# jsyrjala/zraytrace

Measured on AMD Instinct MI355X. Metric: Mrays/s + achieved HBM GB/s, bunny BVH @ 2048², 1024spp, 1/2/4/8 GPUs, higher is better.
Workload: dtype f32

## Files before the change

include/zrt.h:

```cpp
#ifndef ZRT_H
#define ZRT_H

#include <stddef.h>
#include <stdint.h>

#ifdef __cplusplus
extern "C" {
#endif

#define ZRT_ABI_VERSION 2

enum {
  ZRT_OK = 0,
  ZRT_E_INVALID = -1,
  ZRT_E_NOMEM = -2,
  ZRT_E_HIP = -3,
  ZRT_E_UNSUPPORTED = -4,
  ZRT_E_NODEVICE = -5,
  ZRT_E_IO = -6,
  ZRT_E_PARSE = -7
};

enum { ZRT_PRIM_SPHERE = 0, ZRT_PRIM_TRIANGLE = 1 };
enum { ZRT_MAT_LAMBERTIAN = 0, ZRT_MAT_METAL = 1, ZRT_MAT_DIELECTRIC = 2 };
// ... 245 lines not shown
                        const zrt_adaptive* adaptive);
int zrt_ctx_adapt_level(zrt_ctx* ctx, float* dev_tiles, void* hip_stream, zrt_level_info* out);
int zrt_ctx_adapt_samples(zrt_ctx* ctx, uint32_t* per_tile, uint32_t cap_tiles);

typedef int (*zrt_level_fn)(void* user, const float* rgb, const zrt_level_info* info);
int zrt_render_adaptive(const zrt_scene* scene, const zrt_camera* camera, const zrt_params* params,
                        const zrt_adaptive* adaptive, zrt_level_fn on_level, void* user, float* out_rgb,
                        uint32_t* out_samples, zrt_stats* stats);
int zrt_render_adaptive_progress(const zrt_scene* scene, const zrt_camera* camera, const zrt_params* params,
                                 const zrt_adaptive* adaptive, zrt_level_fn on_level, void* user, float* out_rgb,
                                 uint32_t* out_samples, zrt_stats* stats, zrt_scanline* scanlines);

int zrt_debug_adapt_plan(const zrt_params* params, const zrt_adaptive* adaptive, uint32_t* levels,
                         uint32_t cap, uint32_t* n_levels);

int zrt_ctx_accum_variance(zrt_ctx* ctx, float* dev_tiles_var, void* hip_stream);

int zrt_ctx_assemble_plane(zrt_ctx* ctx, const zrt_params* params, const float* dev_gathered,
                           uint32_t stride_tiles, float* dev_frame, void* hip_stream);

typedef struct zrt_variance_plan {
  uint32_t chunk;
  uint32_t k;
  float ik;
  float sc;
} zrt_variance_plan;
int zrt_debug_variance_plan(const zrt_params* params, uint32_t n_samples, zrt_variance_plan* out);

typedef struct zrt_denoise {
  uint32_t iterations;
  float sigma_color;
  float sigma_normal;
  float sigma_albedo;
  float sigma_depth;
  uint32_t reserved[3];
} zrt_denoise;
enum { ZRT_DEFAULT_DENOISE_ITERATIONS = 5u };

int zrt_denoise_defaults(zrt_denoise* out);

int zrt_ctx_features(zrt_ctx* ctx, const zrt_camera* camera, const zrt_params* params,
                     float* dev_features, void* hip_stream);

int zrt_ctx_denoise(zrt_ctx* ctx, const zrt_params* params, const zrt_denoise* dn,
                    const float* dev_frame, const float* dev_features,
                    float* dev_out, void* hip_stream);
int zrt_ctx_denoise_ms(zrt_ctx* ctx, double* ms);

int zrt_render_denoised(const zrt_scene* scene, const zrt_camera* camera, const zrt_params* params,
                        const zrt_adaptive* adaptive, const zrt_denoise* dn, float* out_rgb, float* out_noisy,
                        float* out_features, zrt_stats* stats, double* denoise_ms);

enum { ZRT_DN_DEMODULATE = 1u };

int zrt_denoise_guided_defaults(zrt_denoise* out, uint32_t* flags);

int zrt_ctx_denoise_guided(zrt_ctx* ctx, const zrt_params* params, const zrt_denoise* dn, uint32_t flags,
                           const float* dev_frame, const float* dev_features, const float* dev_variance,
                           float* dev_out, float* dev_out_variance, void* hip_stream);

int zrt_render_denoised_guided(const zrt_scene* scene, const zrt_camera* camera, const zrt_params* params,
                               const zrt_adaptive* adaptive, const zrt_denoise* dn, uint32_t flags, float* out_rgb,
                               float* out_noisy, float* out_features, float* out_variance, zrt_stats* stats,
                               double* denoise_ms);

typedef struct zrt_reproject_plan {
  zrt_vec3 origin;
  zrt_vec3 rn, ru, rv;
  float s;
  uint32_t valid;
} zrt_reproject_plan;
int zrt_debug_reproject_plan(const zrt_camera* prev, const zrt_params* params, zrt_reproject_plan* out);

typedef struct zrt_temporal {
  float alpha_min;
  uint32_t max_history;
  float sigma_normal;
  float sigma_depth;
  uint32_t flags;
  uint32_t reserved[3];
} zrt_temporal;
enum { ZRT_TA_DEMODULATE = 1u };
enum { ZRT_DEFAULT_TEMPORAL_HISTORY = 32u };

int zrt_temporal_defaults(zrt_temporal* out);

int zrt_ctx_temporal(zrt_ctx* ctx, const zrt_camera* camera, const zrt_params* params, const zrt_temporal* tp,
                     const float* dev_frame, const float* dev_features, const float* dev_variance,
                     float* dev_out, float* dev_out_variance, uint32_t* dev_out_len, void* hip_stream);
int zrt_ctx_temporal_reset(zrt_ctx* ctx);
int zrt_ctx_temporal_ms(zrt_ctx* ctx, double* ms);

typedef int (*zrt_frame_fn)(void* user, const float* rgb, uint32_t frame);
int zrt_render_temporal(const zrt_scene* scene, const zrt_camera* cameras, uint32_t n_frames,
                        const zrt_params* params, const zrt_temporal* tp, const zrt_denoise* dn, uint32_t dn_flags,
                        zrt_frame_fn on_frame, void* user, float* out_rgb, zrt_stats* stats);

typedef struct zrt_scene_data zrt_scene_data;

int zrt_scene_load(uint32_t scene_index, const char* assets_dir,
                   zrt_scene_data** out, zrt_camera* camera);
const zrt_scene* zrt_scene_view(const zrt_scene_data* data);
void zrt_scene_free(zrt_scene_data* data);

int zrt_scene_write(const zrt_scene* scene, const zrt_camera* camera, const char* path);
int zrt_scene_read(const char* path, zrt_scene_data** out, zrt_camera* camera);

int zrt_obj_read(const char* path, uint32_t material, zrt_prim** out_prims, uint32_t* n_prims);
void zrt_free(void* p);

int zrt_image_read_png(const char* path, uint32_t* width, uint32_t* height, float** out_pixels);
int zrt_image_write_png(const char* path, const float* rgb, uint32_t width, uint32_t height);
int zrt_image_write_ppm(const char* path, const float* rgb, uint32_t width, uint32_t height);

typedef struct zrt_bvh_node {
  zrt_vec3 min;
  int32_t left;
  zrt_vec3 max;
  int32_t right;
} zrt_bvh_node;

int zrt_bvh_build(const zrt_scene* scene, zrt_bvh_node** out_nodes,
                  uint32_t* n_nodes, uint32_t* max_depth);

int zrt_bvh_build_device(const zrt_scene* scene, uint32_t device, zrt_bvh_node** out_nodes,
                         uint32_t* n_nodes, uint32_t* max_depth);

int zrt_debug_math(int fn, const float* x, const float* y, float* out, uint32_t n, uint32_t device);
int zrt_debug_rng(uint32_t prng, uint64_t key, uint64_t* out, uint32_t n, uint32_t device);
int zrt_debug_division(uint64_t n, uint64_t* counts, uint32_t device);
int zrt_debug_compact(const uint32_t* list, uint32_t n, const uint32_t* tile_done, uint32_t n_tiles,
                      uint32_t* out, uint32_t* count, uint32_t device);
int zrt_debug_lds_plans(const zrt_scene* scene, uint32_t* n_checked);
int zrt_debug_buffer_plans(const zrt_scene* scene, uint32_t legacy, uint32_t* n_checked);
typedef struct zrt_launch_plan {
  uint32_t mode;
  uint32_t kmode;
  uint32_t sampling_loop;
  uint32_t stk16;
  uint32_t wf, pool, qnodes, guard_on;
  uint32_t stack_depth;
  uint32_t stack_rows;
  uint32_t att_rows;
  uint32_t att_rows_per_path;
  uint32_t mats_in_lds;
  uint32_t lds_bytes;
  uint64_t ovf_bytes_per_lane;
} zrt_launch_plan;
int zrt_debug_launch_plan(const zrt_scene* scene, const zrt_params* params, zrt_launch_plan* out);
int zrt_debug_lean_kernel(const zrt_scene* scene, const zrt_camera* camera, const zrt_params* params,
                          uint32_t* lean);
int zrt_debug_qnodes(const zrt_scene* scene, uint64_t* n_checked);
int zrt_debug_octant_offsets(uint32_t stride_f4, uint32_t n_top, uint32_t node_f4);

#ifdef __cplusplus
}
#endif
#endif
```

zraytrace_amd/__init__.py:

```python
from __future__ import annotations

import ctypes as C
import os
from dataclasses import dataclass

import numpy as np

from . import _ffi
from ._ffi import (ZRT_PRNG_XOROSHIRO128, ZRT_PRNG_XOSHIRO256, ZRT_RNG_COUNTER,
                   ZRT_RNG_REFERENCE_STREAM, ZRT_TRAVERSAL_FAST, ZRT_TRAVERSAL_REFERENCE,
                   ZRT_TRAVERSAL_BINARY, ZRT_FLAG_STATS, ZRT_FLAG_NO_SCHEDULE, ZRT_FLAG_SCANLINES, ZRT_FLAG_GUARD,
                   ZRT_DN_DEMODULATE, ZRT_TA_DEMODULATE, ZrtError, check)

REPO = os.path.dirname(os.path.dirname(os.path.abspath(__file__)))
ASSETS = os.path.join(REPO, "assets")

SCENES = {0: "manAndBall", 1: "threeBalls", 2: "bunnyAndBall", 3: "teapotAndBall",
          4: "teapotAndBallCircle", 5: "goat"}


def lib():
    return _ffi.load()


# ... 471 lines not shown
    def debug_counters(self, n: int = 48):
        out = (C.c_uint64 * n)()
        check(lib().zrt_ctx_debug_counters(self._h, out, n))
        return list(out)

    def debug_wave_times(self, cap: int = 1 << 16):
        out = np.zeros(cap, np.uint64)
        n = C.c_uint32()
        check(lib().zrt_ctx_debug_wave_times(self._h, out.ctypes.data_as(C.POINTER(C.c_uint64)), cap, C.byref(n)))
        return out[: 2 * n.value].reshape(-1, 2).copy()

    def debug_schedule(self, cap: int = 1 << 20):
        costs = np.zeros(cap, np.uint32)
        order = np.zeros(cap, np.uint32)
        n = C.c_uint32()
        check(lib().zrt_ctx_debug_schedule(self._h, costs.ctypes.data_as(C.POINTER(C.c_uint32)),
                                           order.ctypes.data_as(C.POINTER(C.c_uint32)), cap, C.byref(n)))
        return costs[: n.value].copy(), order[: n.value].copy()

    def kernel_ms(self) -> float:
        ms = C.c_double()
        check(lib().zrt_ctx_last_kernel_ms(self._h, C.byref(ms)))
        return ms.value

    def close(self):
        if getattr(self, "_h", None):
            lib().zrt_ctx_destroy(self._h)
            self._h = None

    def __del__(self):
        try:
            self.close()
        except Exception:
            pass


def bvh_build(scene):
    view = scene.view if isinstance(scene, LoadedScene) else scene
    nodes = C.POINTER(_ffi.BvhNode)()
    n = C.c_uint32()
    depth = C.c_uint32()
    check(lib().zrt_bvh_build(view, C.byref(nodes), C.byref(n), C.byref(depth)))
    try:
        return nodes_to_numpy(nodes, n.value) + (depth.value,)
    finally:
        lib().zrt_free(C.cast(nodes, C.c_void_p))


def bvh_build_device(scene, device: int = 0):
    view = scene.view if isinstance(scene, LoadedScene) else scene
    nodes = C.POINTER(_ffi.BvhNode)()
    n = C.c_uint32()
    depth = C.c_uint32()
    check(lib().zrt_bvh_build_device(view, device, C.byref(nodes), C.byref(n), C.byref(depth)))
    try:
        return nodes_to_numpy(nodes, n.value) + (depth.value,)
    finally:
        lib().zrt_free(C.cast(nodes, C.c_void_p))


def nodes_to_numpy(nodes, n):
    dt = np.dtype([("min", "<f4", 3), ("left", "<i4"), ("max", "<f4", 3), ("right", "<i4")])
    buf = np.ctypeslib.as_array(C.cast(nodes, C.POINTER(C.c_uint8)), shape=(n * 32,)).copy()
    a = buf.view(dt)
    return a["min"].copy(), a["max"].copy(), a["left"].copy(), a["right"].copy()


def debug_division(n: int = 1 << 30, device: int = 0) -> dict:
    out = (C.c_uint64 * 5)()
    check(lib().zrt_debug_division(n, out, device))
    return dict(zip(("rcp_sqrt_all_2p32", "div", "unit", "inv_dir", "jitter"), (int(v) for v in out)))


def debug_math(fn: int, x, y=None, device: int = 0):
    x = np.ascontiguousarray(x, dtype=np.float32)
    out = np.empty_like(x)
    yp = None
    if y is not None:
        y = np.ascontiguousarray(y, dtype=np.float32)
        yp = y.ctypes.data_as(C.POINTER(C.c_float))
    check(lib().zrt_debug_math(fn, x.ctypes.data_as(C.POINTER(C.c_float)), yp,
                               out.ctypes.data_as(C.POINTER(C.c_float)), x.size, device))
    return out


def debug_rng(prng: int, key: int, n: int, device: int = 0):
    out = np.empty(n, dtype=np.uint64)
    check(lib().zrt_debug_rng(prng, key, out.ctypes.data_as(C.POINTER(C.c_uint64)), n, device))
    return out


def debug_compact(list_, tile_done, fill: int = 0xFFFFFFFF, device: int = 0):
    u32p = C.POINTER(C.c_uint32)
    lst = np.ascontiguousarray(list_, dtype=np.uint32)
    done = np.ascontiguousarray(tile_done, dtype=np.uint32)
    out = np.full(lst.size, fill, dtype=np.uint32)
    count = C.c_uint32()
    check(lib().zrt_debug_compact(lst.ctypes.data_as(u32p), lst.size, done.ctypes.data_as(u32p), done.size,
                                  out.ctypes.data_as(u32p), C.byref(count), device))
    return out, count.value


def read_png(path: str):
    w, h, px = C.c_uint32(), C.c_uint32(), C.POINTER(C.c_float)()
    check(lib().zrt_image_read_png(path.encode(), C.byref(w), C.byref(h), C.byref(px)))
    try:
        return np.ctypeslib.as_array(px, shape=(h.value, w.value, 3)).copy()
    finally:
        lib().zrt_free(px)


def write_png(path: str, image) -> None:
    img = np.ascontiguousarray(image, dtype=np.float32)
    h, w, _ = img.shape
    check(lib().zrt_image_write_png(os.fsencode(path), img.ctypes.data_as(C.POINTER(C.c_float)), w, h))


def write_ppm(path: str, image) -> None:
    img = np.ascontiguousarray(image, dtype=np.float32)
    h, w, _ = img.shape
    check(lib().zrt_image_write_ppm(os.fsencode(path), img.ctypes.data_as(C.POINTER(C.c_float)), w, h))


def debug_lds_plans(scene) -> int:
    view = scene.view if isinstance(scene, LoadedScene) else scene
    n = C.c_uint32()
    check(lib().zrt_debug_lds_plans(view, C.byref(n)))
    return n.value


def debug_buffer_plans(scene, legacy: bool = False) -> int:
    view = scene.view if isinstance(scene, LoadedScene) else scene
    n = C.c_uint32()
    check(lib().zrt_debug_buffer_plans(view, 1 if legacy else 0, C.byref(n)))
    return n.value


def debug_launch_plan(scene, params) -> dict:
    view = scene.view if isinstance(scene, LoadedScene) else scene
    out = _ffi.LaunchPlan()
    p = params.abi()
    check(lib().zrt_debug_launch_plan(view, C.byref(p), C.byref(out)))
    return out.as_dict()


def debug_lean_kernel(scene, camera, params) -> bool:
    view = scene.view if isinstance(scene, LoadedScene) else scene
    out = C.c_uint32()
    p = params.abi()
    check(lib().zrt_debug_lean_kernel(view, C.byref(camera), C.byref(p), C.byref(out)))
    return bool(out.value)


def debug_qnodes(scene) -> int:
    view = scene.view if isinstance(scene, LoadedScene) else scene
    n = C.c_uint64()
    check(lib().zrt_debug_qnodes(view, C.byref(n)))
    return n.value


def debug_octant_offsets(stride_f4: int, n_top: int, node_f4: int = 8) -> None:
    check(lib().zrt_debug_octant_offsets(stride_f4, n_top, node_f4))
```

zraytrace_amd/_ffi.py:

```python
from __future__ import annotations

import ctypes as C
import os

HERE = os.path.dirname(os.path.abspath(__file__))
LIB_PATH = os.environ.get("ZRT_LIB") or os.path.join(HERE, "libzrt.so")

ABI_VERSION = 2
ZRT_OK = 0
ZRT_E_INVALID = -1
ZRT_E_NOMEM = -2
ZRT_E_HIP = -3
ZRT_E_UNSUPPORTED = -4
ZRT_E_NODEVICE = -5
ZRT_E_IO = -6
ZRT_E_PARSE = -7

ZRT_PRIM_SPHERE, ZRT_PRIM_TRIANGLE = 0, 1
ZRT_MAT_LAMBERTIAN, ZRT_MAT_METAL, ZRT_MAT_DIELECTRIC = 0, 1, 2
ZRT_TEX_COLOR, ZRT_TEX_IMAGE = 0, 1
ZRT_RNG_COUNTER, ZRT_RNG_REFERENCE_STREAM = 0, 1
ZRT_PRNG_XOROSHIRO128, ZRT_PRNG_XOSHIRO256 = 0, 1
ZRT_TRAVERSAL_FAST, ZRT_TRAVERSAL_REFERENCE, ZRT_TRAVERSAL_BINARY = 0, 1, 2
ZRT_FLAG_STATS = 1
# ... 123 lines not shown
                ("reserved2", C.c_uint32)]

    def as_dict(self):
        return {name: getattr(self, name) for name, _ in self._fields_ if not name.startswith("reserved")}


LEVEL_FN = C.CFUNCTYPE(C.c_int, C.c_void_p, C.POINTER(C.c_float), C.POINTER(LevelInfo))


class Denoise(C.Structure):
    _fields_ = [("iterations", C.c_uint32), ("sigma_color", C.c_float), ("sigma_normal", C.c_float),
                ("sigma_albedo", C.c_float), ("sigma_depth", C.c_float), ("reserved", C.c_uint32 * 3)]

    def as_dict(self):
        return {name: getattr(self, name) for name, _ in self._fields_ if name != "reserved"}


class VariancePlan(C.Structure):
    _fields_ = [("chunk", C.c_uint32), ("k", C.c_uint32), ("ik", C.c_float), ("sc", C.c_float)]

    def as_dict(self):
        return {name: getattr(self, name) for name, _ in self._fields_}


class ReprojectPlan(C.Structure):
    _fields_ = [("origin", Vec3), ("rn", Vec3), ("ru", Vec3), ("rv", Vec3), ("s", C.c_float), ("valid", C.c_uint32)]


class Temporal(C.Structure):
    _fields_ = [("alpha_min", C.c_float), ("max_history", C.c_uint32), ("sigma_normal", C.c_float),
                ("sigma_depth", C.c_float), ("flags", C.c_uint32), ("reserved", C.c_uint32 * 3)]

    def as_dict(self):
        return {name: getattr(self, name) for name, _ in self._fields_ if name != "reserved"}


FRAME_FN = C.CFUNCTYPE(C.c_int, C.c_void_p, C.POINTER(C.c_float), C.c_uint32)


class BvhNode(C.Structure):
    _fields_ = [("min", Vec3), ("left", C.c_int32), ("max", Vec3), ("right", C.c_int32)]


_P = C.c_void_p
SIGNATURES = [
    ("zrt_render", C.c_int, [C.POINTER(Scene), C.POINTER(Camera), C.POINTER(Params),
                             C.POINTER(C.c_float), C.POINTER(Stats)]),
    ("zrt_render_progress", C.c_int, [C.POINTER(Scene), C.POINTER(Camera), C.POINTER(Params),
                                      C.POINTER(C.c_float), C.POINTER(Stats), C.POINTER(Scanline)]),
    ("zrt_render_multi", C.c_int, [C.POINTER(Scene), C.POINTER(Camera), C.POINTER(Params),
                                   C.POINTER(C.c_uint32), C.c_uint32, C.POINTER(C.c_float), C.POINTER(Stats)]),
    ("zrt_multi_create", C.c_int, [C.POINTER(Scene), C.POINTER(Params), C.POINTER(C.c_uint32), C.c_uint32,
                                   C.POINTER(_P)]),
    ("zrt_multi_render", C.c_int, [_P, C.POINTER(Camera), C.POINTER(Params), C.POINTER(C.c_float),
                                   C.POINTER(Stats)]),
    ("zrt_multi_destroy", C.c_int, [_P]),
    ("zrt_multi_scanlines", C.c_int, [_P, C.POINTER(Scanline), C.c_uint32]),
    ("zrt_multi_frame", C.c_int, [_P, C.POINTER(C.c_float), C.c_uint64]),
    ("zrt_multi_rank_ms", C.c_int, [_P, C.POINTER(C.c_double), C.c_uint32]),
    ("zrt_trace", C.c_int, [C.POINTER(Scene), C.POINTER(Params), C.POINTER(C.c_float), C.c_uint32,
                            C.POINTER(C.c_float), C.POINTER(C.c_int32)]),
    ("zrt_camera_init", C.c_int, [C.POINTER(C.c_float), C.POINTER(C.c_float),
                                  C.POINTER(C.c_float), C.c_float, C.c_float,
                                  C.POINTER(Camera)]),
    ("zrt_last_error", C.c_char_p, []),
    ("zrt_abi_version", C.c_int, []),
    ("zrt_build_info", C.c_char_p, []),
    ("zrt_build_id", C.c_char_p, []),
    ("zrt_ctx_create", C.c_int, [C.POINTER(Scene), C.POINTER(Params), C.POINTER(_P)]),
    ("zrt_ctx_destroy", C.c_int, [_P]),
    ("zrt_ctx_tile_count", C.c_int, [_P, C.POINTER(Params), C.POINTER(C.c_uint32)]),
    ("zrt_ctx_render_tiles", C.c_int, [_P, C.POINTER(Camera), C.POINTER(Params), _P, _P]),
    ("zrt_ctx_assemble", C.c_int, [_P, C.POINTER(Params), _P, _P, _P]),
    ("zrt_ctx_assemble_padded", C.c_int, [_P, C.POINTER(Params), _P, C.c_uint32, _P, _P]),
    ("zrt_ctx_sync", C.c_int, [_P]),
    ("zrt_ctx_scanlines", C.c_int, [_P, C.POINTER(Scanline), C.c_uint32]),
    ("zrt_ctx_stats", C.c_int, [_P, C.POINTER(Stats)]),
    ("zrt_ctx_last_kernel_ms", C.c_int, [_P, C.POINTER(C.c_double)]),
    ("zrt_ctx_debug_counters", C.c_int, [_P, C.POINTER(C.c_uint64), C.c_uint32]),
    ("zrt_ctx_debug_wave_times", C.c_int, [_P, C.POINTER(C.c_uint64), C.c_uint32, C.POINTER(C.c_uint32)]),
    ("zrt_ctx_debug_schedule", C.c_int, [_P, C.POINTER(C.c_uint32), C.POINTER(C.c_uint32), C.c_uint32,
                                         C.POINTER(C.c_uint32)]),
    ("zrt_ctx_accum_begin", C.c_int, [_P, C.POINTER(Camera), C.POINTER(Params)]),
    ("zrt_ctx_accum_pass", C.c_int, [_P, C.c_uint32, _P, _P]),
    ("zrt_ctx_accum_info", C.c_int, [_P, C.POINTER(PassInfo)]),
    ("zrt_render_progressive", C.c_int, [C.POINTER(Scene), C.POINTER(Camera), C.POINTER(Params), C.c_uint32,
                                         PASS_FN, _P, C.POINTER(C.c_float), C.POINTER(Stats)]),
    ("zrt_debug_pass_plan", C.c_int, [C.POINTER(Params), C.c_uint32, C.c_uint32, C.POINTER(PassPlan)]),
    ("zrt_ctx_adapt_begin", C.c_int, [_P, C.POINTER(Camera), C.POINTER(Params), C.POINTER(Adaptive)]),
    ("zrt_ctx_adapt_level", C.c_int, [_P, _P, _P, C.POINTER(LevelInfo)]),
    ("zrt_ctx_adapt_samples", C.c_int, [_P, C.POINTER(C.c_uint32), C.c_uint32]),
    ("zrt_render_adaptive", C.c_int, [C.POINTER(Scene), C.POINTER(Camera), C.POINTER(Params), C.POINTER(Adaptive),
                                      LEVEL_FN, _P, C.POINTER(C.c_float), C.POINTER(C.c_uint32), C.POINTER(Stats)]),
    ("zrt_render_adaptive_progress", C.c_int, [C.POINTER(Scene), C.POINTER(Camera), C.POINTER(Params),
                                               C.POINTER(Adaptive), LEVEL_FN, _P, C.POINTER(C.c_float),
                                               C.POINTER(C.c_uint32), C.POINTER(Stats), C.POINTER(Scanline)]),
    ("zrt_debug_adapt_plan", C.c_int, [C.POINTER(Params), C.POINTER(Adaptive), C.POINTER(C.c_uint32), C.c_uint32,
                                       C.POINTER(C.c_uint32)]),
    ("zrt_ctx_features", C.c_int, [_P, C.POINTER(Camera), C.POINTER(Params), _P, _P]),
    ("zrt_render_denoised", C.c_int, [C.POINTER(Scene), C.POINTER(Camera), C.POINTER(Params), C.POINTER(Adaptive),
                                      C.POINTER(Denoise), C.POINTER(C.c_float), C.POINTER(C.c_float),
                                      C.POINTER(C.c_float), C.POINTER(Stats), C.POINTER(C.c_double)]),
    ("zrt_denoise_defaults", C.c_int, [C.POINTER(Denoise)]),
    ("zrt_ctx_denoise", C.c_int, [_P, C.POINTER(Params), C.POINTER(Denoise), _P, _P, _P, _P]),
    ("zrt_ctx_denoise_ms", C.c_int, [_P, C.POINTER(C.c_double)]),
    ("zrt_ctx_accum_variance", C.c_int, [_P, _P, _P]),
    ("zrt_ctx_assemble_plane", C.c_int, [_P, C.POINTER(Params), _P, C.c_uint32, _P, _P]),
    ("zrt_debug_variance_plan", C.c_int, [C.POINTER(Params), C.c_uint32, C.POINTER(VariancePlan)]),
    ("zrt_denoise_guided_defaults", C.c_int, [C.POINTER(Denoise), C.POINTER(C.c_uint32)]),
    ("zrt_ctx_denoise_guided", C.c_int, [_P, C.POINTER(Params), C.POINTER(Denoise), C.c_uint32, _P, _P, _P, _P, _P,
                                         _P]),
    ("zrt_render_denoised_guided", C.c_int, [C.POINTER(Scene), C.POINTER(Camera), C.POINTER(Params),
                                             C.POINTER(Adaptive), C.POINTER(Denoise), C.c_uint32,
                                             C.POINTER(C.c_float), C.POINTER(C.c_float), C.POINTER(C.c_float),
                                             C.POINTER(C.c_float), C.POINTER(Stats), C.POINTER(C.c_double)]),
    ("zrt_debug_reproject_plan", C.c_int, [C.POINTER(Camera), C.POINTER(Params), C.POINTER(ReprojectPlan)]),
    ("zrt_temporal_defaults", C.c_int, [C.POINTER(Temporal)]),
    ("zrt_ctx_temporal", C.c_int, [_P, C.POINTER(Camera), C.POINTER(Params), C.POINTER(Temporal), _P, _P, _P, _P, _P,
                                   _P, _P]),
    ("zrt_ctx_temporal_reset", C.c_int, [_P]),
    ("zrt_ctx_temporal_ms", C.c_int, [_P, C.POINTER(C.c_double)]),
    ("zrt_render_temporal", C.c_int, [C.POINTER(Scene), C.POINTER(Camera), C.c_uint32, C.POINTER(Params),
                                      C.POINTER(Temporal), C.POINTER(Denoise), C.c_uint32, FRAME_FN, _P,
                                      C.POINTER(C.c_float), C.POINTER(Stats)]),
    ("zrt_scene_load", C.c_int, [C.c_uint32, C.c_char_p, C.POINTER(_P), C.POINTER(Camera)]),
    ("zrt_scene_view", C.POINTER(Scene), [_P]),
    ("zrt_scene_free", None, [_P]),
    ("zrt_scene_write", C.c_int, [C.POINTER(Scene), C.POINTER(Camera), C.c_char_p]),
    ("zrt_scene_read", C.c_int, [C.c_char_p, C.POINTER(_P), C.POINTER(Camera)]),
    ("zrt_obj_read", C.c_int, [C.c_char_p, C.c_uint32, C.POINTER(C.POINTER(Prim)),
                               C.POINTER(C.c_uint32)]),
    ("zrt_free", None, [_P]),
    ("zrt_image_read_png", C.c_int, [C.c_char_p, C.POINTER(C.c_uint32), C.POINTER(C.c_uint32),
                                     C.POINTER(C.POINTER(C.c_float))]),
    ("zrt_image_write_png", C.c_int, [C.c_char_p, C.POINTER(C.c_float), C.c_uint32, C.c_uint32]),
    ("zrt_image_write_ppm", C.c_int, [C.c_char_p, C.POINTER(C.c_float), C.c_uint32, C.c_uint32]),
    ("zrt_bvh_build", C.c_int, [C.POINTER(Scene), C.POINTER(C.POINTER(BvhNode)),
                                C.POINTER(C.c_uint32), C.POINTER(C.c_uint32)]),
    ("zrt_bvh_build_device", C.c_int, [C.POINTER(Scene), C.c_uint32, C.POINTER(C.POINTER(BvhNode)),
                                       C.POINTER(C.c_uint32), C.POINTER(C.c_uint32)]),
    ("zrt_debug_math", C.c_int, [C.c_int, C.POINTER(C.c_float), C.POINTER(C.c_float),
                                 C.POINTER(C.c_float), C.c_uint32, C.c_uint32]),
    ("zrt_debug_rng", C.c_int, [C.c_uint32, C.c_uint64, C.POINTER(C.c_uint64),
                                C.c_uint32, C.c_uint32]),
    ("zrt_debug_division", C.c_int, [C.c_uint64, C.POINTER(C.c_uint64), C.c_uint32]),
    ("zrt_debug_compact", C.c_int, [C.POINTER(C.c_uint32), C.c_uint32, C.POINTER(C.c_uint32), C.c_uint32,
                                    C.POINTER(C.c_uint32), C.POINTER(C.c_uint32), C.c_uint32]),
    ("zrt_debug_lds_plans", C.c_int, [C.POINTER(Scene), C.POINTER(C.c_uint32)]),
    ("zrt_debug_buffer_plans", C.c_int, [C.POINTER(Scene), C.c_uint32, C.POINTER(C.c_uint32)]),
    ("zrt_debug_launch_plan", C.c_int, [C.POINTER(Scene), C.POINTER(Params), C.POINTER(LaunchPlan)]),
    ("zrt_debug_lean_kernel", C.c_int, [C.POINTER(Scene), C.POINTER(Camera), C.POINTER(Params),
                                        C.POINTER(C.c_uint32)]),
    ("zrt_debug_qnodes", C.c_int, [C.POINTER(Scene), C.POINTER(C.c_uint64)]),
    ("zrt_debug_octant_offsets", C.c_int, [C.c_uint32, C.c_uint32, C.c_uint32]),
]

_lib = None


class ZrtError(RuntimeError):
    def __init__(self, code, msg):
        super().__init__(f"zrt error {code}: {msg}")
        self.code = code


def load(path: str = LIB_PATH):
    global _lib
    if _lib is not None and path == LIB_PATH:
        return _lib
    try:
        import torch
    except ImportError:
        pass
    if not os.path.exists(path):
        raise ImportError(
            f"{path} is missing: build the HIP extension first "
            "(python -c 'import __graft_entry__ as g; g.build()'); there is no fallback path")
    lib = C.CDLL(path)
    in_tree = path == os.path.join(HERE, "libzrt.so")
    rebuild = "rebuild it (python -c 'import __graft_entry__ as g; g.build()')"
    lib.zrt_abi_version.restype = C.c_int
    lib.zrt_abi_version.argtypes = []
    abi = lib.zrt_abi_version()
    if abi != ABI_VERSION:
        if in_tree:
            raise ImportError(f"{path} has ABI version {abi}, this binding expects {ABI_VERSION}: {rebuild}")
        if os.environ.get("ZRT_ALLOW_ABI_MISMATCH") != "1":
            raise ImportError(f"ZRT_LIB {path} has ABI version {abi}, this binding expects {ABI_VERSION} "
                              "(set ZRT_ALLOW_ABI_MISMATCH=1 to bind it anyway)")
        import warnings
        warnings.warn(f"ZRT_LIB {path} has ABI version {abi}, this binding expects {ABI_VERSION} "
                      "(bound anyway: ZRT_ALLOW_ABI_MISMATCH=1)")
    for name, restype, argtypes in SIGNATURES:
        if not hasattr(lib, name):
            if in_tree:
                raise ImportError(f"{path} does not export {name} (built from older sources): {rebuild}")
            continue
        fn = getattr(lib, name)
        fn.restype = restype
        fn.argtypes = argtypes
    if path == LIB_PATH:
        _lib = lib
    return lib


def check(rc: int):
    if rc != ZRT_OK:
        raise ZrtError(rc, (load().zrt_last_error() or b"").decode())
    return rc
```

zraytrace_amd/csrc/context.cpp:

```cpp
#include <algorithm>
#include <cmath>
#include <cstdio>
#include <cstdlib>
#include <cstring>

#include "accel_build.hpp"
#include "context.hpp"

namespace zrt {
static const KernelConfig& K = kernel_config();

int check_device(int dev) {
  int count = 0;
  if (hipGetDeviceCount(&count) != hipSuccess || count == 0)
    return fail(ZRT_E_NODEVICE, "no HIP device visible (the HIP path needs an MI355X / gfx950)");
  if (dev < 0 || dev >= count) return fail(ZRT_E_NODEVICE, "device ordinal out of range");
  hipDeviceProp_t prop;
  if (hipGetDeviceProperties(&prop, dev) != hipSuccess) return fail(ZRT_E_NODEVICE, "hipGetDeviceProperties failed");
  if (std::strncmp(prop.gcnArchName, "gfx950", 6) != 0)
    return fail(ZRT_E_NODEVICE, std::string("device is ") + prop.gcnArchName + ", libzrt is built for gfx950 only");
  return ZRT_OK;
}

void flatten_for_device(HostScene* h, const zrt_scene* s, bool use_bvh, int device) {
// ... 40 lines not shown
}

static void fill_tree(KArgs& a, const Scene& s, bool qn) {
  a.wnodes = qn ? s.qnodes.p : s.wnodes.p;
  a.wide_stride = qn ? s.q_stride : s.wide_stride;
  a.node_f4 = qn ? kQuantNodeF4 : 8u;
  a.qleaves = qn ? s.qleaves.p : nullptr;
  a.n_qnodes = qn ? s.q_stride / kQuantNodeF4 : 0u;
  a.n_qleaves = qn ? s.n_qleaves : 0u;
  a.n_top = qn ? s.shape.q_top : s.shape.n_top;
}
static void fill_scene(KArgs& a, const zrt_ctx* c, bool qn, uint32_t stack_depth) {
  const Scene& s = c->scene;
  a.nodes = s.nodes.p;
  a.prims = s.prims.p;
  a.shade = s.shade.p;
  a.mats = s.mats.p;
  a.texels = s.texels.p;
  a.texels8 = s.texels8.p;
  a.n_mats = s.shape.n_mats;
  fill_tree(a, s, qn);
  a.error_flag = reinterpret_cast<uint32_t*>(c->scratch.p + kErrorSlot);
  a.n_list = s.shape.use_bvh ? 0 : s.n_prims;
  a.tri_rcp_fast = s.tri_rcp_fast;
  a.scene_extent = s.scene_extent;
  a.paxis_m = paxis_threshold();
  for (int k = 0; k < 3; ++k) {
    a.tri_c[k] = s.tri_c[k];
    a.tri_h[k] = s.tri_h[k];
    a.root_c[k] = s.root_c[k];
  }
  a.stack_depth = stack_depth;
  a.ref_stack = std::min(s.shape.stack_depth, stack_depth);
  a.leaf_of_slot = s.leaf_of_slot.p;
  a.ref_sph = s.ref_sph.p;
  a.origin_bound = s.origin_bound;
  a.layout = s.layout;
  a.graze_m = s.graze_m;
  a.graze_leaf = s.graze_leaf;
}
void fill_camera(KArgs& a, const zrt_camera* cam, const zrt_params* p) {
  copy3(a.org, cam->origin);
  copy3(a.llc, cam->lower_left_corner);
  copy3(a.hor, cam->horizontal);
  copy3(a.ver, cam->vertical);
  a.f_width = float(p->width);
  a.f_height = float(p->height);
  a.inv_width = 1.0f / a.f_width;
  a.inv_height = 1.0f / a.f_height;
  a.width = p->width;
  a.height = p->height;
  a.xbound = geometry(p).xbound;
}
static void fill_lds(KArgs& a, const LdsPlan& lp) {
  a.lds_rows = lp.stack_rows;
  a.lds_top_off = lp.top_off;
  a.lds_att_off = lp.att_off;
  a.att_lds_rows = lp.att_rows;
  a.lds_mat_off = lp.mat_off;
  a.mats_in_lds = lp.mats_in_lds;
  a.lds_pool_off = lp.pool_off;
  a.lds_state_off = lp.state_off;
}

TracePlan fill_trace(KArgs& a, const zrt_ctx* c, uint32_t traversal) {
  const Scene& s = c->scene;
  const int mode = !s.shape.use_bvh ? 0 : traversal == ZRT_TRAVERSAL_REFERENCE ? 2 : traversal == ZRT_TRAVERSAL_BINARY ? 1 : 3;
  const uint32_t stack_depth = mode == 3 ? std::max(s.shape.wide_stack, s.shape.stack_depth) : s.shape.stack_depth;
  const bool qn = mode == 3 && s.shape.q_ok;
  TracePlan t;
  t.kmode = qn ? 8 : mode;
  t.stk16 = mode == 3 ? fast_stk16(s.shape.n_wide, s.shape.n_nodes) : s.shape.n_nodes < 65536;
  t.lp = plan_lds(qn ? s.shape.q_top : s.shape.n_top, s.shape.n_mats, mode, t.stk16, stack_depth, 0, false, false,
                  ZRT_PRNG_XOROSHIRO128, qn ? kQuantNodeF4 : 8u);
  fill_scene(a, c, qn, stack_depth);
  fill_lds(a, t.lp);
  a.check_origins = 1;
  a.guard = s.shape.guard;
  return t;
}
void trace_rows(KArgs& a, const zrt_ctx* c, const TracePlan& t, uint64_t n_lanes, DevBuf<uint8_t>& ovf, hipStream_t st,
                const char* launch) {
  a.n_lanes = uint32_t(n_lanes);
  const BufNeed need = buffer_need(t.lp, 0, a.stack_depth, n_lanes, n_lanes, t.stk16);
  if (need.ovf_bytes) {
    if (ovf.n < need.ovf_bytes) {
      HIPCHK(hipStreamSynchronize(st));
      ovf.alloc(need.ovf_bytes);
    }
    a.stack_ovf = ovf.p;
  }
  check_buffers(launch, BufNeed{0, need.ovf_bytes}, c->att.n, ovf.n);
  a.att_cap = c->att.n;
  a.ovf_cap = ovf_cap_elems(ovf.n, t.stk16);
}

static bool schedule_tiles(zrt_ctx* c, KArgs& a, uint32_t prng, bool stk16, uint32_t my_tiles, uint32_t grid,
                           hipStream_t st) {
  Probe& pr = c->probe;
  const SceneShape& sh = c->scene.shape;
  const LdsPlan pp = plan_lds(sh.n_top, sh.n_mats, 3, stk16, a.stack_depth, a.max_depth, false, false, prng);
  if (K.mats_lds_only && !pp.mats_in_lds) return false;
  pr.partial.grow(uint64_t(my_tiles) * 64u);
  pr.scratch.grow(kScratchSlots);
  if (pr.tile_cost.n < my_tiles) {
    pr.tile_cost.alloc(my_tiles);
    pr.cost_sorted.alloc(my_tiles);
    pr.tile_order.alloc(my_tiles);
  }
  if (pr.tile_ids_n != my_tiles) {
    std::vector<uint32_t> ids(my_tiles);
    for (uint32_t i = 0; i < my_tiles; ++i) ids[i] = i;
    pr.tile_ids.upload(ids);
    pr.tile_ids_n = my_tiles;
  }
  KArgs pa = a;
  pa.spp = pa.chunk = K.probe_spp;
  pa.n_chunks = 1;
  pa.total_work = my_tiles;
  pa.tile_order = nullptr;
  pa.unit_cost = pr.tile_cost.p;
  pa.partial = pr.partial.p;
  pa.counters = pr.scratch.p;
  pa.work_counter = reinterpret_cast<uint32_t*>(pr.scratch.p + kWorkSlot);
  const uint32_t pgrid = std::max(1u, std::min(grid, (my_tiles + kBlock / 64 - 1) / (kBlock / 64)));
  pa.n_lanes = pgrid * kBlock;
  fill_tree(pa, c->scene, false);
  fill_lds(pa, pp);
  const BufNeed need = buffer_need(pp, a.max_depth, a.stack_depth, pa.n_lanes, pa.n_lanes, stk16);
  if (need.ovf_bytes) {
    if (c->stack_ovf.n < need.ovf_bytes) {
      HIPCHK(hipStreamSynchronize(st));
      c->stack_ovf.alloc(need.ovf_bytes);
    }
    a.stack_ovf = pa.stack_ovf = c->stack_ovf.p;
  }
  if (c->att.n < need.att_elems) {
    HIPCHK(hipStreamSynchronize(st));
    c->att.alloc(need.att_elems);
  }
  a.att = pa.att = c->att.p;
  a.att_cap = pa.att_cap = c->att.n;
  a.ovf_cap = pa.ovf_cap = ovf_cap_elems(c->stack_ovf.n, stk16);
  check_buffers("scheduling probe", need, c->att.n, c->stack_ovf.n);
  HIPCHK(hipMemsetAsync(pr.scratch.p, 0, kScratchSlots * sizeof(unsigned long long), st));
  void* args[] = {&pa};
  HIPCHK(hipLaunchKernel(probe_kernel(prng, stk16), dim3(pgrid), dim3(kBlock), args, pp.bytes, st));
  size_t bytes = 0;
  HIPCHK(sort_tiles(nullptr, &bytes, pr.tile_cost.p, pr.cost_sorted.p, pr.tile_ids.p, pr.tile_order.p, my_tiles, st));
  pr.sort_temp.grow(bytes);
  HIPCHK(sort_tiles(pr.sort_temp.p, &bytes, pr.tile_cost.p, pr.cost_sorted.p, pr.tile_ids.p, pr.tile_order.p, my_tiles,
                    st));
  a.tile_order = pr.tile_order.p;
  return true;
}

int hip_fail(const HipError& e) {
  return fail(ZRT_E_HIP, e.where + ": " + hipGetErrorString(e.err));
}

constexpr const char* kOverflowMsg = "BVH traversal stack overflow (tree deeper than the stack was sized for)";
constexpr const char* kLayoutMsg = "the kernel refused the wide tree: its layout is not the one the kernel decodes";
constexpr const char* kBoundsMsg = "a global attenuation or stack row index past its buffer (STATS bounds check)";
const char* device_error_msg(unsigned long long flag) {
  return (flag & kErrLayout) ? kLayoutMsg : (flag & kErrBounds) ? kBoundsMsg : kOverflowMsg;
}

static int completion_status(Completion& k, bool wait, bool once) {
  if (!k.launched || (k.reported && (once || !wait))) return ZRT_OK;
  if (wait) {
    HIPCHK(hipEventSynchronize(k.done));
  } else if (hipEventQuery(k.done) != hipSuccess) {
    (void)hipGetLastError();
    return ZRT_OK;
  }
  if (*k.err == 0) return ZRT_OK;
  k.reported = true;
  return fail(ZRT_E_UNSUPPORTED, device_error_msg(*k.err));
}
int launch_status(zrt_ctx* c, bool wait) {
  const int rc = completion_status(c->feat.done, wait, true);
  return rc ? rc : completion_status(c->render, wait, false);
}

LaunchTimes launch_times(const EvSet& e) {
  LaunchTimes t{};
  HIPCHK(hipEventElapsedTime(&t.render_ms, e.pre, e.e1));
  HIPCHK(hipEventElapsedTime(&t.schedule_ms, e.pre, e.e0));
  HIPCHK(hipEventElapsedTime(&t.kernel_ms, e.e0, e.e1));
  if (!e.probed) t.schedule_ms = 0.0f;
  return t;
}

void fold_pass_times(zrt_ctx* c, bool wait) {
  AccumRun& r = c->run;
  while (!r.pending.empty()) {
    EvSet& e = r.pending.front();
    if (wait) {
      HIPCHK(hipEventSynchronize(e.e1));
    } else if (hipEventQuery(e.e1) != hipSuccess) {
      (void)hipGetLastError();
      break;
    }
    const LaunchTimes t = launch_times(e);
    r.render_ms += t.render_ms;
    r.sched_ms += t.schedule_ms;
    r.spare.push_back(std::move(e));
    r.pending.erase(r.pending.begin());
  }
}

std::unique_ptr<zrt_ctx> ctx_on_device(const HostScene& h, int device) {
  std::unique_ptr<zrt_ctx> c(new zrt_ctx);
  c->device = device;
  HIPCHK(hipSetDevice(c->device));
  c->stream.create();
  c->ev.create();
  c->render.create();
  hipDeviceProp_t prop;
  HIPCHK(hipGetDeviceProperties(&prop, c->device));
  c->cu_count = prop.multiProcessorCount;
  upload_scene(c->scene, h);
  c->scratch.alloc(kScratchSlots);
  return c;
}

static int assemble(zrt_ctx* c, const zrt_params* p, const float* dev_gathered, uint32_t stride_tiles, float* dev_frame,
             void* hip_stream, uint32_t channels = 3) {
  if (!c || !dev_gathered || !dev_frame) return fail(ZRT_E_INVALID, "null argument");
  const int rc = validate_params(p);
  if (rc) return rc;
  try {
    HIPCHK(hipSetDevice(c->device));
    hipStream_t st = stream_of(c, hip_stream);
    const Geometry g = geometry(p);
    uint32_t total = 0;
    if (stride_tiles) {
      for (uint32_t r = 0; r < p->world_size; ++r)
        if (rank_tiles(g, r, p->world_size) > stride_tiles)
          return fail(ZRT_E_INVALID, "stride_tiles is smaller than a rank's tile count");
      if (uint64_t(stride_tiles) * 64u * p->world_size >= (1ull << 32)) return fail(ZRT_E_UNSUPPORTED, "frame too large");
      total = stride_tiles * 64u * p->world_size;
    } else {
      std::vector<uint32_t> base(p->world_size + 1, 0);
      for (uint32_t r = 0; r < p->world_size; ++r) base[r + 1] = base[r] + rank_tiles(g, r, p->world_size) * 64u;
      c->rank_base.upload(base);
      total = base[p->world_size];
    }
    HIPCHK(hipMemsetAsync(dev_frame, 0, sizeof(float) * channels * size_t(p->width) * p->height, st));
    if (total) {
      HIPCHK((channels == 1 ? launch_assemble_plane : launch_assemble)(
          st, dev_gathered, dev_frame, stride_tiles ? nullptr : c->rank_base.p, p->world_size, g.tiles_x, g.xbound,
          p->height, p->width, total, stride_tiles * 64u, g.n_tiles));
    }
    return ZRT_OK;
  }
  ZRT_CATCH_ALL
}

int params_fit_ctx(const zrt_ctx* c, const zrt_params* p) {
  if (int(p->device) != c->device)
    return fail(ZRT_E_INVALID, "params->device differs from the device the context was created on");
  if ((p->bounded_volume_hierarchy != 0 && c->scene.n_prims > 10) != c->scene.shape.use_bvh)
    return fail(ZRT_E_INVALID,
                "params->bounded_volume_hierarchy implies another preprocessSufraces decision (raytrace.zig:124-133) "
                "than the one the context was built with");
  return ZRT_OK;
}

namespace {
struct LaunchEnv {
  bool debug = false;
  uint32_t wf_thresh = 48;
  uint32_t sync = 0;
  bool order_cache = true;
  bool auto_sync = true;
  bool cap_rows = false;
  double row_cap = 1.0;
};
LaunchEnv read_launch_env() {
  LaunchEnv v;
  v.debug = std::getenv("ZRT_DEBUG_LAUNCH") != nullptr;
  if (const char* e = std::getenv("ZRT_WF_THRESH")) v.wf_thresh = uint32_t(std::max(1, std::min(64, std::atoi(e))));
  if (const char* e = std::getenv("ZRT_SYNC")) v.sync = std::max(1u, uint32_t(std::atoi(e)));
  const char* oc = std::getenv("ZRT_ORDER_CACHE");
  v.order_cache = !(oc && std::atoi(oc) == 0);
  const char* as = std::getenv("ZRT_AUTO_SYNC");
  v.auto_sync = !v.sync && !(as && std::atoi(as) == 0);
  if (const char* e = std::getenv("ZRT_DEBUG_ROW_CAP")) {
    v.cap_rows = true;
    v.row_cap = std::atof(e);
  }
  return v;
}

struct Frame {
  const zrt_camera* cam;
  const zrt_params* p;
  float* dev_tiles;
  hipStream_t st;
  bool run_pass, first, adapt, diag, cam_inside;
  zrt_pass_plan pass;
  Geometry g;
  uint32_t my_tiles;
  LaunchPlan plan;
  void* kfn;
};
struct FrameSize {
  int per_cu;
  uint32_t grid, n_act, work;
  uint64_t n_lanes, n_paths;
  BufNeed need;
};

int plan_frame(zrt_ctx* c, const zrt_camera* cam, const zrt_params* p, float* dev_tiles, void* hip_stream,
               bool run_pass, uint32_t n_samples, Frame* f) {
  if (!c || !cam || !dev_tiles) return fail(ZRT_E_INVALID, "null argument");
  int rc = plan_pass(p, run_pass ? c->run.done : 0u, run_pass ? n_samples : (p ? p->samples_per_pixel : 0u), &f->pass);
  if (rc) return rc;
  rc = params_fit_ctx(c, p);
  if (rc) return rc;
  HIPCHK(hipSetDevice(c->device));
  rc = launch_status(c, false);
  if (rc) return rc;
  f->cam = cam;
  f->p = p;
  f->dev_tiles = dev_tiles;
  f->st = stream_of(c, hip_stream);
  f->run_pass = run_pass;
  f->first = !run_pass || c->run.passes == 0;
  f->adapt = run_pass && c->adapt.on;
  f->diag = (p->flags & ZRT_FLAG_STATS) != 0;
  f->g = geometry(p);
  f->my_tiles = rank_tiles(f->g, p->rank, p->world_size);
  f->plan = plan_launch(c->scene.shape, p);
  f->cam_inside = camera_inside(cam, c->scene.root_c, c->scene.origin_bound);
  f->kfn = select_kernel(f->plan.kmode, p->prng, f->diag, f->plan.stk16, lean_launch(f->plan, f->diag, f->cam_inside));
  return ZRT_OK;
}

int size_frame(const zrt_ctx* c, const Frame& f, FrameSize* z) {
  HIPCHK(hipOccupancyMaxActiveBlocksPerMultiprocessor(&z->per_cu, f.kfn, kBlock, f.plan.lp.bytes));
  z->per_cu = std::max(1, std::min(z->per_cu, 8));
  z->n_act = f.adapt ? c->adapt.n_active : f.my_tiles;
  z->work = uint32_t(uint64_t(z->n_act) * f.pass.pass_chunks);
  z->grid = std::max(1u, std::min(uint32_t(c->cu_count) * uint32_t(z->per_cu), (z->work + (kBlock / 64) - 1) / (kBlock / 64)));
  z->n_lanes = uint64_t(z->grid) * kBlock;
  z->n_paths = f.plan.pool ? uint64_t(z->grid) * K.block_paths : z->n_lanes;
  if (z->n_paths >= (1ull << 32)) return fail(ZRT_E_UNSUPPORTED, "too many paths");
  z->need = buffer_need(f.plan.lp, f.p->max_depth, f.plan.stack_depth, z->n_paths, z->n_lanes, f.plan.stk16);
  if (z->need.att_elems * sizeof(uint32_t) > (16ull << 30))
    return fail(ZRT_E_UNSUPPORTED, "max_depth too large for the per-lane attenuation stack");
  return ZRT_OK;
}

void prepare_buffers(zrt_ctx* c, const Frame& f, const FrameSize& z) {
  c->partial.grow(uint64_t(f.my_tiles) * 64u * f.pass.pass_chunks);
  c->att.grow(z.need.att_elems);
  if (z.need.ovf_bytes) c->stack_ovf.grow(z.need.ovf_bytes);
  if (f.first)
    HIPCHK(hipMemsetAsync(c->scratch.p, 0, kScratchSlots * sizeof(unsigned long long), f.st));
  else
    HIPCHK(hipMemsetAsync(c->scratch.p + kWorkSlot, 0, sizeof(unsigned long long), f.st));
  if (f.run_pass && f.first) {
    HIPCHK(hipMemsetAsync(c->run.accum.p, 0, c->run.accum.n * sizeof(float4), f.st));
    if (f.adapt) HIPCHK(hipMemsetAsync(c->adapt.tile_done.p, 0, c->adapt.tile_done.n * sizeof(uint32_t), f.st));
  }
}

void rotate_events(zrt_ctx* c) {
  AccumRun& r = c->run;
  fold_pass_times(c, false);
  if (r.spare.empty()) {
    r.spare.emplace_back();
    r.spare.back().create();
  }
  r.pending.push_back(std::move(c->ev));
  c->ev = std::move(r.spare.back());
  r.spare.pop_back();
}

KArgs fill_args(const zrt_ctx* c, const Frame& f, const FrameSize& z, const LaunchEnv& env) {
  const LaunchPlan& P = f.plan;
  KArgs a{};
  fill_scene(a, c, P.qn, P.stack_depth);
  fill_camera(a, f.cam, f.p);
  fill_lds(a, P.lp);
  a.att = c->att.p;
  a.partial = c->partial.p;
  a.counters = c->scratch.p;
  a.work_counter = reinterpret_cast<uint32_t*>(c->scratch.p + kWorkSlot);
  a.color_scale = 1.0f / float(f.pass.samples_after);
  a.spp = f.pass.pass_samples;
  a.max_depth = f.p->max_depth;
  a.tiles_x = f.g.tiles_x;
  a.rank = f.p->rank;
  a.world = f.p->world_size;
  a.total_work = z.work;
  a.guard = P.guard_on ? c->scene.shape.guard : 0.0f;
  a.check_origins = f.cam_inside ? 0u : 1u;
  if (z.need.ovf_bytes) a.stack_ovf = c->stack_ovf.p;
  a.n_lanes = uint32_t(z.n_lanes);
  a.n_paths = uint32_t(z.n_paths);
  if (K.mats_lds_only && P.kmode == 3 && !P.lp.mats_in_lds) a.n_mats = 0u;
  a.seed_mix = f.p->seed * 0x9E3779B97F4A7C15ULL + f.pass.key_offset;
  a.chunk = f.pass.chunk;
  a.n_chunks = f.pass.pass_chunks;
  a.wf_thresh = env.wf_thresh;
  a.sync = env.sync ? env.sync : P.mode == 0 ? f.pass.chunk : K.sync_samples;
  a.n_slots = f.my_tiles * 64u;
  if (env.debug)
    std::fprintf(stderr, "zrt launch: mode %d stk16 %d grid %u (%d blocks/CU x %d CUs) lds %zu B "
                 "(stack rows %u, top nodes %u @%u, att rows %u @%u, mats %u @%u)\n", P.mode, int(P.stk16), z.grid,
                 z.per_cu, c->cu_count, P.lp.bytes, P.lp.stack_rows, a.n_top, P.lp.top_off, P.lp.att_rows, P.lp.att_off,
                 P.lp.mats_in_lds ? c->scene.shape.n_mats : 0u, P.lp.mat_off);
  return a;
}

bool choose_order(zrt_ctx* c, const Frame& f, const FrameSize& z, const LaunchEnv& env, KArgs& a) {
  const zrt_params* p = f.p;
  Probe& pr = c->probe;
  HIPCHK(hipEventRecord(c->ev.pre, f.st));
  bool schedule =
      f.plan.mode == 3 && !(p->flags & ZRT_FLAG_NO_SCHEDULE) && p->samples_per_pixel >= 128 && f.my_tiles >= 2;
  bool order_hit = false;
  if (schedule && !f.first) {
    schedule = c->run.ordered;
    if (schedule) a.tile_order = pr.tile_order.p;
  } else if (schedule) {
    const OrderKey key{*f.cam, p->width, p->height, p->max_depth, p->rank, p->world_size, p->traversal,
                       f.plan.guard_on ? 1u : 0u, f.my_tiles};
    order_hit = env.order_cache && pr.order_valid && std::memcmp(&key, &pr.order_key, sizeof(key)) == 0;
    if (order_hit) {
      a.tile_order = pr.tile_order.p;
    } else {
      pr.order_valid = false;
      schedule = schedule_tiles(c, a, p->prng, f.plan.stk16, f.my_tiles, z.grid, f.st);
      pr.order_key = key;
      pr.order_valid = schedule;
    }
  }
  if (f.run_pass && f.first) c->run.ordered = schedule;
  if (f.adapt) {
    uint32_t* list = c->adapt.active[c->adapt.cur].p;
    if (f.first && schedule)
      HIPCHK(hipMemcpyAsync(list, pr.tile_order.p, size_t(f.my_tiles) * sizeof(uint32_t), hipMemcpyDeviceToDevice, f.st));
    a.tile_order = list;
  }
  c->ev.probed = schedule && f.first && !order_hit;
  return schedule;
}

void optional_outputs(zrt_ctx* c, const Frame& f, const FrameSize& z, const LaunchEnv& env, bool schedule, KArgs& a) {
  a.sync_probe = schedule && f.plan.kmode == 3 && env.auto_sync ? c->probe.scratch.p : nullptr;
  if (f.p->flags & ZRT_FLAG_SCANLINES) {
    const size_t n = size_t(f.p->height) * 3;
    c->scanlines.grow(n);
    if (f.first) HIPCHK(hipMemsetAsync(c->scanlines.p, 0, n * sizeof(unsigned long long), f.st));
    a.scanlines = c->scanlines.p;
  }
  if (K.profile) {
    c->wave_times.grow(2ull * z.grid * (kBlock / 64));
    a.wave_times = c->wave_times.p;
  }
  check_buffers("render launch", z.need, c->att.n, c->stack_ovf.n);
  a.att = c->att.p;
  if (z.need.ovf_bytes) a.stack_ovf = c->stack_ovf.p;
  a.att_cap = c->att.n;
  a.ovf_cap = ovf_cap_elems(c->stack_ovf.n, f.plan.stk16);
  if (f.diag && env.cap_rows) {
    a.att_cap = uint64_t(double(a.att_cap) * env.row_cap);
    a.ovf_cap = uint64_t(double(a.ovf_cap) * env.row_cap);
  }
}

void enqueue(zrt_ctx* c, const Frame& f, const FrameSize& z, KArgs& a) {
  const zrt_params* p = f.p;
  const Geometry& g = f.g;
  const uint32_t n_chunks = f.pass.pass_chunks, n_slots = f.my_tiles * 64u;
  unsigned long long* err = c->scratch.p + kErrorSlot;
  HIPCHK(hipEventRecord(c->ev.e0, f.st));
  if (z.work > 0) {
    void* args[] = {&a};
    HIPCHK(hipLaunchKernel(f.kfn, dim3(z.grid), dim3(kBlock), args, f.plan.lp.bytes, f.st));
  }
  HIPCHK(hipEventRecord(c->ev.e1, f.st));
  if (!f.run_pass) {
    if (f.my_tiles > 0)
      HIPCHK(launch_finalize(f.st, c->partial.p, f.dev_tiles, n_slots, n_chunks, p->world_size, p->rank, g.tiles_x,
                             g.xbound, p->height, a.color_scale, err));
    return;
  }
  AccumRun& r = c->run;
  HIPCHK(hipMemsetAsync(r.metrics.p, 0, kMetricWords * sizeof(unsigned long long), f.st));
  const uint32_t q_chunks = n_chunks - (f.pass.last_chunk < f.pass.chunk ? 1u : 0u);
  const float prev_scale = r.done ? 1.0f / float(r.done) : 0.0f;
  if (f.adapt) {
    AdaptRun& ad = c->adapt;
    const uint32_t decide = ad.k >= 1 && ad.k + 1 < ad.levels.size() ? 1u : 0u;
    HIPCHK(hipMemsetAsync(ad.active_count.p, 0, sizeof(uint32_t), f.st));
    if (z.n_act > 0) {
      HIPCHK(launch_resolve(f.st, c->partial.p, r.accum.p, f.dev_tiles, ad.active[ad.cur].p, z.n_act, f.my_tiles,
                            n_chunks, p->world_size, p->rank, g.tiles_x, g.xbound, p->height, prev_scale, a.color_scale,
                            q_chunks, ad.a.tolerance, decide, f.pass.samples_after, ad.tile_done.p, err, r.metrics.p));
      HIPCHK(launch_compact(f.st, ad.active[ad.cur].p, z.n_act, ad.tile_done.p, ad.active[ad.cur ^ 1u].p,
                            ad.active_count.p));
    }
    HIPCHK(hipMemcpyAsync(ad.count_host.get(), ad.active_count.p, sizeof(uint32_t), hipMemcpyDeviceToHost, f.st));
  } else if (f.my_tiles > 0) {
    HIPCHK(launch_accumulate(f.st, c->partial.p, r.accum.p, f.dev_tiles, n_slots, n_chunks, p->world_size, p->rank,
                             g.tiles_x, g.xbound, p->height, prev_scale, a.color_scale, q_chunks, err, r.metrics.p));
  }
  HIPCHK(hipMemcpyAsync(r.metrics_host.get(), r.metrics.p, kMetricWords * sizeof(unsigned long long), hipMemcpyDeviceToHost,
                        f.st));
}

void finish(zrt_ctx* c, const Frame& f, const FrameSize& z, const KArgs& a, bool schedule) {
  HIPCHK(hipMemcpyAsync(c->render.err.get(), c->scratch.p + kErrorSlot, sizeof(unsigned long long), hipMemcpyDeviceToHost,
                        f.st));
  HIPCHK(hipEventRecord(c->render.done, f.st));
  c->render.launched = true;
  c->render.reported = false;
  LastLaunch l;
  l.g = f.g;
  l.height = f.p->height;
  l.rank = f.p->rank;
  l.world = f.p->world_size;
  l.tiles = f.my_tiles;
  uint64_t pixels = 0;
  for_rank_tiles(f.g, l.height, l.rank, l.world,
                 [&pixels](uint32_t, uint32_t w, uint32_t h, uint32_t) { pixels += uint64_t(w) * h; });
  l.pixels = uint32_t(pixels);
  l.spp = f.pass.samples_after;
  l.stats = f.diag;
  l.qn = f.plan.qn;
  l.run = f.run_pass;
  l.adapt = f.adapt;
  l.scheduled = schedule;
  l.mode = f.plan.mode;
  l.loop = int(reported_loop(f.plan.kmode));
  l.guard = a.guard;
  l.scanline_rows = (f.p->flags & ZRT_FLAG_SCANLINES) ? f.p->height : 0u;
  l.n_waves = K.profile ? z.grid * (kBlock / 64) : 0u;
  c->last = l;
  if (f.run_pass) {
    c->run.done = f.pass.samples_after;
    c->run.passes += 1;
    c->run.pass_samples = f.pass.pass_samples;
  } else {
    c->run.live = false;
  }
}
}

int launch_frame(zrt_ctx* c, const zrt_camera* cam, const zrt_params* p, float* dev_tiles, void* hip_stream,
                 bool run_pass, uint32_t n_samples) {
  try {
    Frame f{};
    int rc = plan_frame(c, cam, p, dev_tiles, hip_stream, run_pass, n_samples, &f);
    if (rc) return rc;
    FrameSize z{};
    rc = size_frame(c, f, &z);
    if (rc) return rc;
    const LaunchEnv env = read_launch_env();
    prepare_buffers(c, f, z);
    if (run_pass && !f.first) rotate_events(c);
    KArgs a = fill_args(c, f, z, env);
    const bool schedule = choose_order(c, f, z, env, a);
    optional_outputs(c, f, z, env, schedule, a);
    enqueue(c, f, z, a);
    finish(c, f, z, a, schedule);
    return ZRT_OK;
  }
  ZRT_CATCH_ALL
}
}

using zrt::fail;

int zrt_abi_version(void) { return ZRT_ABI_VERSION; }

const char* zrt_build_info(void) {
  return "libzrt: HIP path for gfx950 (MI355X); persistent wave64 path-tracing kernel; -ffp-contract=off";
}

int zrt_ctx_create(const zrt_scene* scene, const zrt_params* params, zrt_ctx** out) {
  if (!out) return fail(ZRT_E_INVALID, "out is null");
  *out = nullptr;
  int rc = zrt::validate_scene(scene);
  if (rc) return rc;
  if (!params) return fail(ZRT_E_INVALID, "params is null");
  try {
    const bool use_bvh = params->bounded_volume_hierarchy != 0 && scene->n_prims > 10;
    int n_dev = 0;
    const bool gpus = hipGetDeviceCount(&n_dev) == hipSuccess && n_dev > 0;
    if (gpus) {
      rc = zrt::check_device(int(params->device));
      if (rc) return rc;
    }
    const bool have_dev = gpus && int(params->device) < n_dev;
    zrt::HostScene h;
    zrt::flatten_for_device(&h, scene, use_bvh, have_dev ? int(params->device) : -1);
    rc = zrt::check_device(int(params->device));
    if (rc) return rc;
    *out = zrt::ctx_on_device(h, int(params->device)).release();
    return ZRT_OK;
  }
  ZRT_CATCH_ALL
}

int zrt_ctx_destroy(zrt_ctx* ctx) {
  if (!ctx) return ZRT_OK;
  (void)hipSetDevice(ctx->device);
  if (ctx->stream) (void)hipStreamSynchronize(ctx->stream);
  delete ctx;
  return ZRT_OK;
}

int zrt_ctx_tile_count(const zrt_ctx* ctx, const zrt_params* params, uint32_t* n_tiles) {
  (void)ctx;
  if (!n_tiles) return fail(ZRT_E_INVALID, "null argument");
  const int rc = zrt::validate_params(params);
  if (rc) return rc;
  *n_tiles = zrt::rank_tiles(zrt::geometry(params), params->rank, params->world_size);
  return ZRT_OK;
}

int zrt_ctx_render_tiles(zrt_ctx* c, const zrt_camera* cam, const zrt_params* p, float* dev_tiles,
                         void* hip_stream) {
  return zrt::launch_frame(c, cam, p, dev_tiles, hip_stream, false, 0);
}

int zrt_ctx_stats(zrt_ctx* c, zrt_stats* out) {
  if (!c || !out) return fail(ZRT_E_INVALID, "null argument");
  if (!c->render.launched) return fail(ZRT_E_INVALID, "zrt_ctx_stats before any zrt_ctx_render_tiles");
  try {
    const zrt::Scene& s = c->scene;
    const zrt::LastLaunch& l = c->last;
    HIPCHK(hipSetDevice(c->device));
    HIPCHK(hipEventSynchronize(c->render.done));
    unsigned long long h[zrt::kScratchSlots] = {0};
    HIPCHK(hipMemcpy(h, c->scratch.p, sizeof(h), hipMemcpyDeviceToHost));
    if (l.scanline_rows) {
      std::vector<unsigned long long> rows(size_t(l.scanline_rows) * 3);
      HIPCHK(hipMemcpy(rows.data(), c->scanlines.p, rows.size() * sizeof(unsigned long long), hipMemcpyDeviceToHost));
      for (size_t y = 0; y < l.scanline_rows; ++y) {
        h[zrt::kDepthHits] += rows[3 * y];
        h[zrt::kReflections] += rows[3 * y + 1];
        h[zrt::kBackground] += rows[3 * y + 2];
      }
    }
    std::memset(out, 0, sizeof(*out));
    out->recursion_depth_hits = h[zrt::kDepthHits];
    out->reflections = h[zrt::kReflections];
    out->background_hits = h[zrt::kBackground];
    const uint64_t samples = l.adapt ? c->adapt.samples : uint64_t(l.pixels) * l.spp;
    out->rays_processed = l.stats ? h[zrt::kRays] : samples + h[zrt::kReflections] - h[zrt::kDepthHits];
    out->node_visits = h[zrt::kNodes];
    out->prim_tests = h[zrt::kTriTests] + h[zrt::kSphereTests];
    out->sphere_tests = h[zrt::kSphereTests];
    out->shade_fetches = h[zrt::kShades];
    out->texel_fetches = h[zrt::kTexels];
    out->leaf_visits = h[zrt::kLeaves];
    out->order_replays = h[zrt::kReplays];
    uint32_t bt = uint32_t(h[zrt::kExcessTri]), bs = uint32_t(h[zrt::kExcessSph]);
    std::memcpy(&out->box_excess_max_triangle, &bt, 4);
    std::memcpy(&out->box_excess_max_sphere, &bs, 4);
    out->box_excess_hits = h[zrt::kExcessHits];
    out->node_bytes = l.mode == 3 ? (l.qn ? 64 : 128) : 32;
    out->wide_nodes = s.shape.n_wide;
    out->sampling_loop = uint32_t(l.loop);
    out->guard = l.guard;
    out->texel_bytes = s.texel_bytes;
    out->pixels_processed = l.pixels;
    out->samples_processed = samples;
    out->preprocess_ms = s.preprocess_ms;
    out->upload_ms = s.upload_ms;
    const zrt::LaunchTimes t = zrt::launch_times(c->ev);
    out->render_ms = t.render_ms;
    out->schedule_ms = t.schedule_ms;
    if (l.run) {
      zrt::fold_pass_times(c, true);
      out->render_ms = c->run.render_ms + t.render_ms;
      out->schedule_ms = float(c->run.sched_ms + t.schedule_ms);
    }
    out->used_bvh = s.shape.use_bvh ? 1 : 0;
    out->bvh_nodes = s.shape.n_nodes;
    out->bvh_max_depth = s.bvh_depth;
    out->n_gpus = 1;
    return zrt::launch_status(c, true);
  }
  ZRT_CATCH_ALL
}

int zrt_ctx_sync(zrt_ctx* c) {
  if (!c) return fail(ZRT_E_INVALID, "null argument");
  try {
    HIPCHK(hipSetDevice(c->device));
    return zrt::launch_status(c, true);
  }
  ZRT_CATCH_ALL
}

int zrt_ctx_last_kernel_ms(zrt_ctx* c, double* ms) {
  if (!c || !ms) return fail(ZRT_E_INVALID, "null argument");
  if (!c->render.launched) return fail(ZRT_E_INVALID, "no kernel launched on this context yet");
  try {
    HIPCHK(hipSetDevice(c->device));
    HIPCHK(hipEventSynchronize(c->ev.e1));
    *ms = zrt::launch_times(c->ev).kernel_ms;
    return zrt::launch_status(c, true);
  }
  ZRT_CATCH_ALL
}

namespace zrt {
int add_scanlines(zrt_ctx* c, zrt_scanline* out, uint32_t height) {
  const LastLaunch& l = c->last;
  if (!c->render.launched || l.scanline_rows == 0)
    return fail(ZRT_E_INVALID, "the last launch did not count scanlines (ZRT_FLAG_SCANLINES)");
  if (height != l.scanline_rows) return fail(ZRT_E_INVALID, "height differs from the last launch's");
  HIPCHK(hipSetDevice(c->device));
  HIPCHK(hipEventSynchronize(c->render.done));
  std::vector<unsigned long long> rows(size_t(height) * 3);
// ... 54 lines not shown
```

zraytrace_amd/csrc/context.hpp:

```cpp
#pragma once
#include <hip/hip_runtime_api.h>

#include <cstring>
#include <memory>
#include <string>
#include <utility>
#include <vector>

#include "host.hpp"

namespace zrt {
struct HipError {
  hipError_t err;
  std::string where;
};

#define HIPCHK(expr)                                                       \
  do {                                                                     \
    const hipError_t e_ = (expr);                                          \
    if (e_ != hipSuccess) throw ::zrt::HipError{e_, std::string(#expr)};          \
  } while (0)

template <class T>
struct DevBuf {
  T* p = nullptr;
  size_t n = 0;
  DevBuf() = default;
  DevBuf(const DevBuf&) = delete;
  DevBuf& operator=(const DevBuf&) = delete;
  DevBuf(DevBuf&& o) noexcept : p(o.p), n(o.n) {
    o.p = nullptr;
    o.n = 0;
  }
  ~DevBuf() { release(); }
  void release() {
    if (p) (void)hipFree(p);
    p = nullptr;
    n = 0;
  }
  void alloc(size_t count) {
    release();
    if (count == 0) count = 1;
    HIPCHK(hipMalloc(&p, count * sizeof(T)));
    n = count;
  }
  void grow(size_t count) {
    if (n < count) alloc(count);
  }
  void upload(const std::vector<T>& v) {
    alloc(v.size());
    if (!v.empty()) HIPCHK(hipMemcpy(p, v.data(), v.size() * sizeof(T), hipMemcpyHostToDevice));
  }
};

template <class H, hipError_t (*Destroy)(H)>
struct Handle {
  H h = nullptr;
  Handle() = default;
  Handle(Handle&& o) noexcept : h(std::exchange(o.h, nullptr)) {}
  Handle& operator=(Handle&& o) noexcept {
    std::swap(h, o.h);
    return *this;
  }
  ~Handle() {
    if (h) (void)Destroy(h);
  }
  operator H() const { return h; }
};
struct Event : Handle<hipEvent_t, hipEventDestroy> {
  void create(unsigned flags = hipEventDefault) {
    if (!h) HIPCHK(hipEventCreateWithFlags(&h, flags));
  }
};
struct Stream : Handle<hipStream_t, hipStreamDestroy> {
  void create() {
    if (!h) HIPCHK(hipStreamCreateWithFlags(&h, hipStreamDefault));
  }
};

template <class T>
struct Pinned : Handle<void*, hipHostFree> {
  void alloc(size_t count = 1) {
    if (h) return;
    HIPCHK(hipHostMalloc(&h, count * sizeof(T), hipHostMallocDefault));
    std::memset(h, 0, count * sizeof(T));
  }
  T* get() const { return static_cast<T*>(h); }
  T& operator*() const { return *get(); }
  T& operator[](size_t i) const { return get()[i]; }
};

struct EvSet {
  Event pre, e0, e1;
  bool probed = false;
  void create() {
    pre.create();
    e0.create();
    e1.create();
  }
};

struct Completion {
  Event done;
  Pinned<unsigned long long> err;
  bool launched = false;
  bool reported = false;
  void create() {
    done.create(hipEventDisableTiming);
    err.alloc();
  }
};

struct Scene {
  SceneShape shape;
  uint32_t n_prims = 0, bvh_depth = 0, wide_stride = 0;
  std::vector<uint32_t> slot_to_prim;
  DevBuf<float4> wnodes;
  DevBuf<float4> qnodes, qleaves;
  uint32_t q_stride = 0, n_qleaves = 0;
  DevBuf<float4> nodes, prims, shade;
  DevBuf<DevMaterial> mats;
  DevBuf<float> texels;
  DevBuf<uint32_t> texels8;
  DevBuf<uint32_t> leaf_of_slot;
  DevBuf<uint8_t> ref_sph;
  float root_c[3] = {0.0f, 0.0f, 0.0f}, origin_bound = 0.0f;
  uint32_t layout = 0;
  float graze_m = 0x1p-18f, graze_leaf = 0x1p-18f;
  uint32_t texel_bytes = 0;
  uint32_t tri_rcp_fast = 1;
  float scene_extent = 1.0f;
  float tri_c[3] = {0.0f, 0.0f, 0.0f}, tri_h[3] = {0.0f, 0.0f, 0.0f};
  double preprocess_ms = 0, upload_ms = 0;
};

struct OrderKey {
  zrt_camera cam;
  uint32_t width, height, max_depth, rank, world_size, traversal, guard_on, tiles;
};
static_assert(sizeof(OrderKey) == sizeof(zrt_camera) + 8 * sizeof(uint32_t), "OrderKey is compared bitwise: no padding");
struct Probe {
  DevBuf<float4> partial;
  DevBuf<unsigned long long> scratch;
  DevBuf<uint32_t> tile_cost, tile_ids, cost_sorted, tile_order;
  DevBuf<uint8_t> sort_temp;
  uint32_t tile_ids_n = 0;
  OrderKey order_key{};
  bool order_valid = false;
};

struct LastLaunch {
  Geometry g{};
  uint32_t height = 0, rank = 0, world = 1, tiles = 0, pixels = 0, spp = 0;
  bool stats = false, qn = false, run = false, adapt = false, scheduled = false;
  int mode = 0, loop = 0;
  float guard = 0.0f;
  uint32_t scanline_rows = 0;
  uint32_t n_waves = 0;
};

struct AccumRun {
  bool live = false;
  zrt_camera cam{};
  zrt_params p{};
  uint32_t done = 0;
  uint32_t passes = 0;
  bool ordered = false;
  uint32_t pass_samples = 0;
  DevBuf<float4> accum;
  DevBuf<unsigned long long> metrics;
  Pinned<unsigned long long> metrics_host;
  std::vector<EvSet> pending, spare;
  double render_ms = 0, sched_ms = 0;
};

struct AdaptRun {
  bool on = false;
  zrt_adaptive a{};
  std::vector<uint32_t> levels;
  uint32_t k = 0;
  uint32_t n_active = 0;
  uint32_t cur = 0;
  uint64_t samples = 0;
  float* tiles = nullptr;
  DevBuf<uint32_t> active[2], tile_done, active_count;
  Pinned<uint32_t> count_host;
};

struct StepTimer {
  Event e0, e1;
  bool launched = false;
};
struct DenoiseState {
  DevBuf<float4> buf[2];
  StepTimer timer;
};
struct TemporalState {
  DevBuf<float4> hist[2], feat[2];
  DevBuf<uint32_t> len[2];
  uint32_t cur = 0, width = 0, height = 0, demod = 0;
  bool live = false;
  zrt_camera cam{};
  StepTimer timer;
};
struct VariancePlan {
  DevBuf<float2> dev;
  std::vector<float2> host;
};
struct FeatureState {
  DevBuf<uint8_t> ovf;
  DevBuf<uint32_t> slot_prim;
  Completion done;
};
}

struct zrt_ctx {
  int device = 0;
  int cu_count = 0;
  zrt::Stream stream;
  zrt::Scene scene;
  zrt::DevBuf<uint32_t> att;
  zrt::DevBuf<uint8_t> stack_ovf;
  zrt::DevBuf<unsigned long long> scratch;
  zrt::DevBuf<float4> partial;
  zrt::DevBuf<uint32_t> rank_base;
  zrt::DevBuf<unsigned long long> wave_times;
  zrt::DevBuf<unsigned long long> scanlines;
  zrt::Probe probe;
  zrt::EvSet ev;
  zrt::Completion render;
  zrt::LastLaunch last;
  zrt::AccumRun run;
  zrt::AdaptRun adapt;
  zrt::DenoiseState dn;
  zrt::TemporalState ta;
  zrt::VariancePlan var;
  zrt::FeatureState feat;
};

namespace zrt {
int check_device(int dev);
int hip_fail(const HipError& e);
void flatten_for_device(HostScene* h, const zrt_scene* s, bool use_bvh, int device);
std::unique_ptr<zrt_ctx> ctx_on_device(const HostScene& h, int device);
int add_scanlines(zrt_ctx* c, zrt_scanline* out, uint32_t height);

inline hipStream_t stream_of(const zrt_ctx* c, void* hip_stream) {
  return hip_stream ? static_cast<hipStream_t>(hip_stream) : hipStream_t(c->stream);
}
int params_fit_ctx(const zrt_ctx* c, const zrt_params* p);
int launch_frame(zrt_ctx* c, const zrt_camera* cam, const zrt_params* p, float* dev_tiles, void* hip_stream,
                 bool run_pass, uint32_t n_samples);
int launch_status(zrt_ctx* c, bool wait);
const char* device_error_msg(unsigned long long flag);
struct LaunchTimes {
  float render_ms, schedule_ms, kernel_ms;
};
LaunchTimes launch_times(const EvSet& e);
void fold_pass_times(zrt_ctx* c, bool wait);
void fill_camera(KArgs& a, const zrt_camera* cam, const zrt_params* p);
inline void copy3(float dst[3], const zrt_vec3& v) {
  dst[0] = v.x;
  dst[1] = v.y;
  dst[2] = v.z;
}
struct TracePlan {
  int kmode = 0;
  bool stk16 = false;
  LdsPlan lp;
};
TracePlan fill_trace(KArgs& a, const zrt_ctx* c, uint32_t traversal);
void trace_rows(KArgs& a, const zrt_ctx* c, const TracePlan& t, uint64_t n_lanes, DevBuf<uint8_t>& ovf, hipStream_t st,
                const char* launch);
}

#define ZRT_CATCH_ALL                                  \
  catch (const ::zrt::HipError& e) {                   \
    return ::zrt::hip_fail(e);                         \
  }                                                    \
  ZRT_CATCH_HOST
```

zraytrace_amd/csrc/debug_device.cpp:

```cpp
#include <algorithm>
#include <cstdlib>

#include "context.hpp"

using zrt::fail;

int zrt_ctx_debug_counters(zrt_ctx* c, uint64_t* out, uint32_t n) {
  if (!c || !out) return fail(ZRT_E_INVALID, "null argument");
  if (!c->render.launched) return fail(ZRT_E_INVALID, "no kernel launched on this context yet");
  try {
    HIPCHK(hipSetDevice(c->device));
    HIPCHK(hipEventSynchronize(c->render.done));
    unsigned long long h[zrt::kScratchSlots] = {0};
    HIPCHK(hipMemcpy(h, c->scratch.p, sizeof(h), hipMemcpyDeviceToHost));
    for (uint32_t i = 0; i < n && i < uint32_t(zrt::kScratchSlots); ++i) out[i] = h[i];
    return ZRT_OK;
  }
  ZRT_CATCH_ALL
}

int zrt_ctx_debug_wave_times(zrt_ctx* c, uint64_t* out, uint32_t cap, uint32_t* n_waves) {
  if (!c || !n_waves) return fail(ZRT_E_INVALID, "null argument");
  try {
    HIPCHK(hipSetDevice(c->device));
    if (c->render.launched) HIPCHK(hipEventSynchronize(c->render.done));
    *n_waves = c->last.n_waves;
    const size_t n = std::min<size_t>(cap / 2, *n_waves);
    if (n && out) HIPCHK(hipMemcpy(out, c->wave_times.p, 2 * n * sizeof(uint64_t), hipMemcpyDeviceToHost));
    return ZRT_OK;
  }
  ZRT_CATCH_ALL
}

int zrt_ctx_debug_schedule(zrt_ctx* c, uint32_t* costs, uint32_t* order, uint32_t cap, uint32_t* n_tiles) {
  if (!c || !n_tiles) return fail(ZRT_E_INVALID, "null argument");
  if (!c->render.launched) return fail(ZRT_E_INVALID, "no kernel launched on this context yet");
  try {
    HIPCHK(hipSetDevice(c->device));
    HIPCHK(hipEventSynchronize(c->render.done));
    *n_tiles = c->last.scheduled ? c->probe.tile_ids_n : 0u;
    const size_t n = std::min<size_t>(cap, *n_tiles);
    if (n && costs) HIPCHK(hipMemcpy(costs, c->probe.tile_cost.p, n * sizeof(uint32_t), hipMemcpyDeviceToHost));
    if (n && order) HIPCHK(hipMemcpy(order, c->probe.tile_order.p, n * sizeof(uint32_t), hipMemcpyDeviceToHost));
    return ZRT_OK;
  }
  ZRT_CATCH_ALL
}

int zrt_trace(const zrt_scene* scene, const zrt_params* params, const float* rays, uint32_t n_rays, float* out_t,
              int32_t* out_prim) {
  if (!params || (n_rays && (!rays || !out_t || !out_prim))) return fail(ZRT_E_INVALID, "null argument");
  int rc = zrt::validate_scene(scene);
  if (rc) return rc;
  if (params->traversal > ZRT_TRAVERSAL_BINARY) return fail(ZRT_E_INVALID, "unknown traversal");
  rc = zrt::check_device(int(params->device));
  if (rc) return rc;
  if (n_rays == 0) return ZRT_OK;
  try {
    const bool use_bvh = params->bounded_volume_hierarchy != 0 && scene->n_prims > 10;
    zrt::HostScene h;
    zrt::flatten_for_device(&h, scene, use_bvh, int(params->device));
    std::unique_ptr<zrt_ctx> c = zrt::ctx_on_device(h, int(params->device));
    const uint32_t grid = (n_rays + zrt::kBlock - 1) / zrt::kBlock;
    const uint64_t n_lanes = uint64_t(grid) * zrt::kBlock;
    zrt::DevBuf<float> d_rays, d_t;
    zrt::DevBuf<int32_t> d_slot;
    d_rays.alloc(6ull * n_rays);
    d_t.alloc(n_rays);
    d_slot.alloc(n_rays);
    HIPCHK(hipMemcpy(d_rays.p, rays, sizeof(float) * 6ull * n_rays, hipMemcpyHostToDevice));
    HIPCHK(hipMemset(c->scratch.p, 0, zrt::kScratchSlots * sizeof(unsigned long long)));
    zrt::KArgs a{};
    const zrt::TracePlan t = zrt::fill_trace(a, c.get(), params->traversal);
    if (std::getenv("ZRT_DEBUG_NO_GUARD")) a.guard = 0.0f;
    zrt::trace_rows(a, c.get(), t, n_lanes, c->stack_ovf, c->stream, "trace launch");
    void* fn = zrt::trace_kernel_ptr(t.kmode, t.stk16);
    const float* rp = d_rays.p;
    float* tp = d_t.p;
    int32_t* sp = d_slot.p;
    uint32_t nn = n_rays;
    void* args[] = {&a, &rp, &nn, &tp, &sp};
    HIPCHK(hipLaunchKernel(fn, dim3(grid), dim3(zrt::kBlock), args, t.lp.bytes, c->stream));
    HIPCHK(hipStreamSynchronize(c->stream));
    unsigned long long err = 0;
    HIPCHK(hipMemcpy(&err, c->scratch.p + zrt::kErrorSlot, sizeof(err), hipMemcpyDeviceToHost));
    if (err) return fail(ZRT_E_UNSUPPORTED, zrt::device_error_msg(err));
    std::vector<int32_t> slot(n_rays);
    HIPCHK(hipMemcpy(out_t, d_t.p, sizeof(float) * n_rays, hipMemcpyDeviceToHost));
    HIPCHK(hipMemcpy(slot.data(), d_slot.p, sizeof(int32_t) * n_rays, hipMemcpyDeviceToHost));
    for (uint32_t i = 0; i < n_rays; ++i)
      out_prim[i] = slot[i] < 0 ? -1 : int32_t(c->scene.slot_to_prim[size_t(slot[i])]);
    return ZRT_OK;
  }
  ZRT_CATCH_ALL
}

int zrt_debug_math(int fn, const float* x, const float* y, float* out, uint32_t n, uint32_t device) {
  if (!x || !out) return fail(ZRT_E_INVALID, "null argument");
  int rc = zrt::check_device(int(device));
  if (rc) return rc;
  try {
    HIPCHK(hipSetDevice(int(device)));
    zrt::DevBuf<float> dx, dy, dout;
    dx.alloc(n);
    dout.alloc(n);
    HIPCHK(hipMemcpy(dx.p, x, n * sizeof(float), hipMemcpyHostToDevice));
    if (y) {
      dy.alloc(n);
      HIPCHK(hipMemcpy(dy.p, y, n * sizeof(float), hipMemcpyHostToDevice));
    }
    HIPCHK(zrt::launch_debug_math(fn, dx.p, y ? dy.p : nullptr, dout.p, n));
    HIPCHK(hipDeviceSynchronize());
    HIPCHK(hipMemcpy(out, dout.p, n * sizeof(float), hipMemcpyDeviceToHost));
    return ZRT_OK;
  }
  ZRT_CATCH_ALL
}

int zrt_debug_division(uint64_t n, uint64_t* counts, uint32_t device) {
  if (!counts) return fail(ZRT_E_INVALID, "null argument");
  int rc = zrt::check_device(int(device));
  if (rc) return rc;
  try {
    HIPCHK(hipSetDevice(int(device)));
    zrt::DevBuf<unsigned long long> d;
    d.alloc(5);
    HIPCHK(hipMemset(d.p, 0, 5 * sizeof(unsigned long long)));
    HIPCHK(zrt::launch_debug_division(n, d.p));
    HIPCHK(hipDeviceSynchronize());
    HIPCHK(hipMemcpy(counts, d.p, 5 * sizeof(uint64_t), hipMemcpyDeviceToHost));
    return ZRT_OK;
  }
  ZRT_CATCH_ALL
}

int zrt_debug_compact(const uint32_t* list, uint32_t n, const uint32_t* tile_done, uint32_t n_tiles, uint32_t* out,
                      uint32_t* count, uint32_t device) {
  if (!list || !tile_done || !out || !count) return fail(ZRT_E_INVALID, "null argument");
  if (n == 0) return fail(ZRT_E_INVALID, "compact: an empty list");
  for (uint32_t i = 0; i < n; ++i)
    if (list[i] >= n_tiles) return fail(ZRT_E_INVALID, "compact: a list entry is not below n_tiles");
  int rc = zrt::check_device(int(device));
  if (rc) return rc;
  try {
    HIPCHK(hipSetDevice(int(device)));
    zrt::DevBuf<uint32_t> d_list, d_done, d_out, d_count;
    d_list.alloc(n);
    d_done.alloc(n_tiles);
    d_out.alloc(n);
    d_count.alloc(1);
    HIPCHK(hipMemcpy(d_list.p, list, size_t(n) * sizeof(uint32_t), hipMemcpyHostToDevice));
    HIPCHK(hipMemcpy(d_done.p, tile_done, size_t(n_tiles) * sizeof(uint32_t), hipMemcpyHostToDevice));
    HIPCHK(hipMemcpy(d_out.p, out, size_t(n) * sizeof(uint32_t), hipMemcpyHostToDevice));
    HIPCHK(hipMemset(d_count.p, 0, sizeof(uint32_t)));
    HIPCHK(zrt::launch_compact(nullptr, d_list.p, n, d_done.p, d_out.p, d_count.p));
    HIPCHK(hipDeviceSynchronize());
    HIPCHK(hipMemcpy(out, d_out.p, size_t(n) * sizeof(uint32_t), hipMemcpyDeviceToHost));
    HIPCHK(hipMemcpy(count, d_count.p, sizeof(uint32_t), hipMemcpyDeviceToHost));
    return ZRT_OK;
  }
  ZRT_CATCH_ALL
}

int zrt_debug_rng(uint32_t prng, uint64_t key, uint64_t* out, uint32_t n, uint32_t device) {
  if (!out) return fail(ZRT_E_INVALID, "null argument");
  int rc = zrt::check_device(int(device));
  if (rc) return rc;
// ... 12 lines not shown
```

zraytrace_amd/csrc/debug_plans.cpp:

```cpp
#include <cmath>
#include <cstring>
#include <string>

#include "accel_build.hpp"
#include "host.hpp"

using zrt::fail;

int zrt_debug_pass_plan(const zrt_params* params, uint32_t done, uint32_t n_samples, zrt_pass_plan* out) {
  if (!out) return fail(ZRT_E_INVALID, "null argument");
  return zrt::plan_pass(params, done, n_samples, out);
}

int zrt_debug_adapt_plan(const zrt_params* params, const zrt_adaptive* adaptive, uint32_t* levels, uint32_t cap,
                         uint32_t* n_levels) {
  if (!n_levels || (cap && !levels)) return fail(ZRT_E_INVALID, "null argument");
  std::vector<uint32_t> L;
  const int rc = zrt::plan_adapt(params, adaptive, &L);
  if (rc) return rc;
  *n_levels = uint32_t(L.size());
  for (uint32_t k = 0; k < cap && k < L.size(); ++k) levels[k] = L[k];
  return ZRT_OK;
}

int zrt_debug_variance_plan(const zrt_params* params, uint32_t n_samples, zrt_variance_plan* out) {
  if (!out) return fail(ZRT_E_INVALID, "null argument");
  return zrt::plan_variance(params, n_samples, out);
}

int zrt_debug_reproject_plan(const zrt_camera* prev, const zrt_params* params, zrt_reproject_plan* out) {
  if (!out) return fail(ZRT_E_INVALID, "null argument");
  return zrt::plan_reproject(prev, params, out);
}

int zrt_debug_octant_offsets(uint32_t stride_f4, uint32_t n_top, uint32_t node_f4) {
  try {
    zrt::check_octant_offsets(stride_f4, n_top, node_f4);
    return ZRT_OK;
  }
  ZRT_CATCH_HOST
}

int zrt_debug_lds_plans(const zrt_scene* scene, uint32_t* n_checked) {
  if (!n_checked) return fail(ZRT_E_INVALID, "null argument");
  *n_checked = 0;
  int rc = zrt::validate_scene(scene);
  if (rc) return rc;
  try {
    zrt::HostScene h;
    zrt::flatten_scene(&h, scene, scene->n_prims > 10, -1, scene->n_prims > 10 ? 1 : 0);
    const uint32_t n_mats = uint32_t(h.mats.size());
    const uint32_t ref_depth = h.use_bvh ? h.bvh_depth + 2 : 0;
    std::string where;
    for (int mode : {0, 1, 2, 3}) {
      for (int loop = 0; loop < (mode == 3 ? 3 : 1); ++loop) {
        for (bool stk16 : {true, false}) {
          for (uint32_t prng : {uint32_t(ZRT_PRNG_XOROSHIRO128), uint32_t(ZRT_PRNG_XOSHIRO256)}) {
            for (uint32_t depth : {0u, 1u, 2u, 5u, 20u, 50u}) {
              for (uint32_t nf4 : {8u, 4u}) {
                if (nf4 == 4u && (loop != 2 || !h.q_ok)) continue;
                for (uint32_t cap : {zrt::stack_rows_cap(), 1u, 2u, 4u}) {
                  const bool capped = cap != zrt::stack_rows_cap();
                  if (capped && !(mode == 3 && stk16)) continue;
                  const uint32_t sd = mode == 3 ? std::max(h.wide_stack, ref_depth) : ref_depth;
                  where = "mode " + std::to_string(mode) + " loop " + std::to_string(loop) + " stk16 " +
                          std::to_string(int(stk16)) + " prng " + std::to_string(prng) + " depth " +
                          std::to_string(depth) + " node_f4 " + std::to_string(nf4) +
                          (capped ? " stack rows capped at " + std::to_string(cap) : std::string());
                  try {
                    (void)zrt::plan_lds(nf4 == 4u ? h.q_top : h.n_top, n_mats, mode, stk16, sd, depth, loop == 1,
                                        loop == 2, prng, nf4, cap);
                  } catch (const zrt::Error& e) {
                    throw zrt::Error(e.code, std::string(e.what()) + " (" + where + ")");
                  }
                  ++*n_checked;
                }
              }
            }
          }
        }
      }
    }
    return ZRT_OK;
  }
  ZRT_CATCH_HOST
}

int zrt_debug_buffer_plans(const zrt_scene* scene, uint32_t legacy, uint32_t* n_checked) {
  if (!n_checked) return fail(ZRT_E_INVALID, "null argument");
  *n_checked = 0;
  int rc = zrt::validate_scene(scene);
  if (rc) return rc;
  if (scene->n_prims <= 10) return ZRT_OK;
  try {
    zrt::HostScene h;
    zrt::flatten_scene(&h, scene, true, -1, 1);
    const uint32_t n_mats = uint32_t(h.mats.size());
    const uint32_t sd = std::max(h.wide_stack, h.bvh_depth + 2);
    for (int loop = 0; loop < 3; ++loop) {
      for (bool stk16 : {true, false}) {
        for (uint32_t prng : {uint32_t(ZRT_PRNG_XOROSHIRO128), uint32_t(ZRT_PRNG_XOSHIRO256)}) {
          for (uint32_t depth : {0u, 1u, 2u, 4u, 5u, 6u, 13u, 20u, 50u}) {
            for (uint32_t nf4 : {8u, 4u}) {
              if (nf4 == 4u && (loop != 2 || !h.q_ok)) continue;
              for (uint32_t grid : {64u, 1536u, 2048u}) {
               for (uint32_t cap : {zrt::stack_rows_cap(), 1u, 2u, 4u}) {
                const bool capped = cap != zrt::stack_rows_cap();
                if (capped && !stk16) continue;
                const std::string where = "loop " + std::to_string(loop) + " stk16 " + std::to_string(int(stk16)) +
                                          " prng " + std::to_string(prng) + " depth " + std::to_string(depth) +
                                          " node_f4 " + std::to_string(nf4) + " grid " + std::to_string(grid) +
                                          (capped ? " stack rows capped at " + std::to_string(cap) : std::string());
                const zrt::LdsPlan lp = zrt::plan_lds(nf4 == 4u ? h.q_top : h.n_top, n_mats, 3, stk16, sd, depth,
                                                      loop == 1, loop == 2, prng, nf4, cap);
                const uint64_t n_lanes = uint64_t(grid) * zrt::kBlock;
                const uint64_t n_paths = loop == 2 ? uint64_t(grid) * zrt::kernel_config().block_paths : n_lanes;
                const zrt::BufNeed rn = zrt::buffer_need(lp, depth, sd, n_paths, n_lanes, stk16);
                const zrt::LdsPlan pp = zrt::plan_lds(h.n_top, n_mats, 3, stk16, sd, depth, false, false, prng, 8, cap);
                const zrt::BufNeed pn = zrt::buffer_need(pp, depth, sd, n_lanes, n_lanes, stk16);
                uint64_t att = rn.att_elems, ovf = std::max(rn.ovf_bytes, pn.ovf_bytes);
                if (!legacy) att = std::max(att, pn.att_elems);
                try {
                  zrt::check_buffers("scheduling probe", pn, att, ovf);
                  zrt::check_buffers("render launch", rn, att, ovf);
                } catch (const zrt::Error& e) {
                  throw zrt::Error(e.code, std::string(e.what()) + " (" + where + ")");
                }
                ++*n_checked;
               }
              }
            }
          }
        }
      }
    }
    return ZRT_OK;
  }
  ZRT_CATCH_HOST
}

int zrt_debug_launch_plan(const zrt_scene* scene, const zrt_params* params, zrt_launch_plan* out) {
  if (!params || !out) return fail(ZRT_E_INVALID, "null argument");
  std::memset(out, 0, sizeof(*out));
  int rc = zrt::validate_scene(scene);
  if (rc) return rc;
  if (params->traversal > ZRT_TRAVERSAL_BINARY) return fail(ZRT_E_INVALID, "unknown traversal");
  try {
    const bool use_bvh = params->bounded_volume_hierarchy != 0 && scene->n_prims > 10;
    zrt::HostScene h;
    zrt::flatten_scene(&h, scene, use_bvh, -1);
    const zrt::LaunchPlan P = zrt::plan_launch(zrt::shape_of(h), params);
    out->mode = uint32_t(P.mode);
    out->kmode = uint32_t(P.kmode);
    out->sampling_loop = zrt::reported_loop(P.kmode);
    out->stk16 = P.stk16;
    out->wf = P.wf;
    out->pool = P.pool;
    out->qnodes = P.qn;
    out->guard_on = P.guard_on;
    out->stack_depth = P.stack_depth;
    out->stack_rows = P.lp.stack_rows;
    out->att_rows = P.lp.att_rows;
    out->att_rows_per_path = zrt::att_rows_per_path(P.lp, params->max_depth);
    out->mats_in_lds = P.lp.mats_in_lds;
    out->lds_bytes = uint32_t(P.lp.bytes);
    out->ovf_bytes_per_lane = zrt::buffer_need(P.lp, params->max_depth, P.stack_depth, 1, 1, P.stk16).ovf_bytes;
    return ZRT_OK;
  }
  ZRT_CATCH_HOST
}

int zrt_debug_lean_kernel(const zrt_scene* scene, const zrt_camera* camera, const zrt_params* params, uint32_t* lean) {
  if (!camera || !params || !lean) return fail(ZRT_E_INVALID, "null argument");
  *lean = 0;
  int rc = zrt::validate_scene(scene);
  if (rc) return rc;
  if (params->traversal > ZRT_TRAVERSAL_BINARY) return fail(ZRT_E_INVALID, "unknown traversal");
  try {
    const bool use_bvh = params->bounded_volume_hierarchy != 0 && scene->n_prims > 10;
    zrt::HostScene h;
    zrt::flatten_scene(&h, scene, use_bvh, -1);
    const zrt::LaunchPlan P = zrt::plan_launch(zrt::shape_of(h), params);
    *lean = zrt::lean_launch(P, (params->flags & ZRT_FLAG_STATS) != 0,
                             zrt::camera_inside(camera, h.root_c, h.origin_bound))
                ? 1u
                : 0u;
    return ZRT_OK;
  }
  ZRT_CATCH_HOST
}

int zrt_debug_qnodes(const zrt_scene* scene, uint64_t* n_checked) {
  if (!n_checked) return fail(ZRT_E_INVALID, "null argument");
  *n_checked = 0;
  int rc = zrt::validate_scene(scene);
  if (rc) return rc;
  if (scene->n_prims <= 10) return fail(ZRT_E_INVALID, "no BVH for <= 10 surfaces (raytrace.zig:124-133)");
  try {
    zrt::HostScene h;
    zrt::flatten_scene(&h, scene, true, -1, 1);
    if (!h.q_ok) return fail(ZRT_E_UNSUPPORTED, "the encoder refused this tree (a non-finite plane)");
    const uint32_t nn = h.q_stride / zrt::kQuantNodeF4, nw = h.wide_stride / 8u;
    if (nn != nw) return fail(ZRT_E_UNSUPPORTED, "compressed and full trees differ in node count");
    auto bad = [](const std::string& what, uint32_t o, uint32_t i, int k) {
      return fail(ZRT_E_UNSUPPORTED, what + " (octant " + std::to_string(o) + ", node " + std::to_string(i) + ", slot " +
                                         std::to_string(k) + ")");
    };
    for (uint32_t o = 0; o < 8; ++o) {
      for (uint32_t i = 0; i < nn; ++i) {
        const float4* F = &h.wn[size_t(o) * h.wide_stride + 8u * i];
        uint32_t W[16];
        std::memcpy(W, &h.qn[size_t(o) * h.q_stride + zrt::kQuantNodeF4 * i], sizeof(W));
        float org[3], step[3];
        std::memcpy(org, W, 12);
        for (int a = 0; a < 3; ++a) step[a] = std::ldexp(1.0f, int((W[3] >> (8 * a)) & 0xffu) - 127);
        int32_t fr[4], qr[4], fb[4];
        std::memcpy(fr, &F[6], 16);
        std::memcpy(fb, &F[7], 16);
        std::memcpy(qr, &W[10], 16);
        for (int k = 0; k < 4; ++k) {
          const float* fn = reinterpret_cast<const float*>(F);
          const bool empty = qr[k] == zrt::kEmptyRef;
          for (int a = 0; a < 3 && !empty; ++a) {
            const double qn = double((W[4 + a] >> (8 * k)) & 0xffu), qf = double((W[7 + a] >> (8 * k)) & 0xffu);
            const double dn = double(org[a]) + qn * double(step[a]), df = double(org[a]) + qf * double(step[a]);
            if (double(float(dn)) != dn || double(float(df)) != df) return bad("a plane does not decode exactly", o, i, k);
            const bool neg = (o >> a) & 1u;
            const double full_n = fn[4 * a + k], full_f = fn[4 * (3 + a) + k];
            if (neg ? !(dn >= full_n && df <= full_f) : !(dn <= full_n && df >= full_f))
              return bad("a decoded box does not contain the full node's", o, i, k);
          }
          if (!empty && qr[k] >= 0 && qr[k] != fr[k]) return bad("an inner child ref differs", o, i, k);
          if (!empty && qr[k] < 0) {
            const bool sph = qr[k] < -zrt::kSphereSlotBias;
            const uint32_t L = uint32_t(-(sph ? qr[k] + zrt::kSphereSlotBias : qr[k]) - 1);
            if (size_t(L) * zrt::kLeafRecF4 + 1 >= h.ql.size()) return bad("a leaf record index past the records", o, i, k);
            const float4 mn = h.ql[zrt::kLeafRecF4 * size_t(L)], mx = h.ql[zrt::kLeafRecF4 * size_t(L) + 1];
            const float m[3] = {mn.x, mn.y, mn.z}, M[3] = {mx.x, mx.y, mx.z};
            for (int a = 0; a < 3; ++a) {
              const bool neg = (o >> a) & 1u;
              const float full_n = fn[4 * a + k], full_f = fn[4 * (3 + a) + k];
              const float rn = neg ? M[a] : m[a], rf = neg ? m[a] : M[a];
              if (std::memcmp(&rn, &full_n, 4) || std::memcmp(&rf, &full_f, 4)) return bad("a leaf record's box differs", o, i, k);
            }
            int32_t ra, rb;
            std::memcpy(&ra, &mn.w, 4);
            std::memcpy(&rb, &mx.w, 4);
            const int32_t full_a = sph ? fr[k] + zrt::kSphereSlotBias : fr[k];
            if (ra != full_a || rb != fb[k] || sph != (fr[k] < -zrt::kSphereSlotBias))
              return bad("a leaf record's refs differ", o, i, k);
          }
          ++*n_checked;
        }
      }
    }
    return ZRT_OK;
  }
  ZRT_CATCH_HOST
}
```

zraytrace_amd/csrc/host.hpp:

```cpp
#pragma once
#include <hip/hip_runtime_api.h>

#include <cstddef>
#include <cstdint>
#include <functional>
#include <new>
#include <vector>

#include "denoise.hpp"
#include "kernels.hpp"
#include "temporal.hpp"
#include "zrt.hpp"

namespace zrt {
struct Geometry {
  uint32_t xbound, tiles_x, tiles_y, n_tiles;
};

struct HostScene {
  bool use_bvh = false;
  uint32_t n_prims = 0, n_nodes = 0, bvh_depth = 0;
  uint32_t n_wide = 0, n_leaves = 0, wide_stack = 0, wide_stride = 0, n_top = 0, n_mats = 0;
  uint32_t texel_bytes = 0;
  uint32_t tri_rcp_fast = 1;
  uint32_t has_dielectric = 0, has_image_texture = 0;
  float scene_extent = 0.0f;
  float tri_c[3] = {0.0f, 0.0f, 0.0f}, tri_h[3] = {0.0f, 0.0f, 0.0f};
  float root_c[3] = {0.0f, 0.0f, 0.0f}, origin_bound = 0.0f;
  uint32_t layout = 0;
  float graze_m = 0x1p-18f;
  float graze_leaf = 0x1p-18f;
  float guard = 0.0f;
  std::vector<uint8_t> ref_sph;
  std::vector<float4> nodes, wn, prims, shade;
  std::vector<float4> qn, ql;
  bool q_ok = false;
  uint32_t q_stride = 0;
  uint32_t q_top = 0;
  std::vector<DevMaterial> mats;
  std::vector<float> tex;
  std::vector<uint32_t> tex8;
  std::vector<uint32_t> slot_to_prim;
  std::vector<uint32_t> leaf_of_slot;
  double preprocess_ms = 0;
  bool device_bvh_failed = false;
};

struct LdsPlan {
  uint32_t stack_rows = 0, top_off = 0, att_off = 0, att_rows = 0, mat_off = 0, mats_in_lds = 0, pool_off = 0;
  uint32_t state_off = 0;
  size_t bytes = 0, budget = 0;
  size_t stack_b = 0, top_b = 0, pool_b = 0, state_b = 0, att_b = 0, mats_b = 0;
};
constexpr size_t kLdsPerBlockMax = 160u << 10;

struct BufNeed {
  uint64_t att_elems = 0;
  uint64_t ovf_bytes = 0;
};

struct SceneShape {
  bool use_bvh = false, q_ok = false;
  uint32_t n_nodes = 0, n_wide = 0, wide_stack = 0, stack_depth = 0, n_top = 0, q_top = 0, n_mats = 0;
  float guard = 0.0f;
  bool tri_rcp_fast = false, has_dielectric = true, has_image_texture = true;
};

struct LaunchPlan {
  int mode = 0;
  int kmode = 0;
  bool stk16 = false, wf = false, pool = false, qn = false, guard_on = false;
  bool lean = false;
  uint32_t node_f4 = 8, stack_depth = 0;
  LdsPlan lp;
};

double now_ms();
int validate_scene(const zrt_scene* s);
int validate_params(const zrt_params* p);
Geometry geometry(const zrt_params* p);
uint32_t rank_tiles(const Geometry& g, uint32_t rank, uint32_t world);
void for_rank_tiles(const Geometry& g, uint32_t height, uint32_t rank, uint32_t world,
                    const std::function<void(uint32_t lt, uint32_t w, uint32_t h, uint32_t y0)>& f);
float paxis_threshold();
void check_octant_offsets(uint32_t stride_f4, uint32_t n_top, uint32_t node_f4);
bool want_qnodes(uint32_t n_wide);
uint32_t qtop_levels();
constexpr uint32_t kNoRowsCap = 0xffffffffu;
uint32_t stack_rows_cap();
bool fast_stk16(uint32_t n_wide, uint32_t n_nodes);
LdsPlan plan_lds(uint32_t n_top, uint32_t n_mats, int mode, bool stk16, uint32_t stack_depth, uint32_t max_depth,
                 bool wf, bool pool, uint32_t prng, uint32_t node_f4 = 8, uint32_t rows_cap = stack_rows_cap());
uint32_t att_rows_per_path(const LdsPlan& lp, uint32_t max_depth);
BufNeed buffer_need(const LdsPlan& lp, uint32_t max_depth, uint32_t stack_depth, uint64_t n_paths, uint64_t n_lanes,
                    bool stk16);
void check_buffers(const char* launch, const BufNeed& need, uint64_t att_elems, uint64_t ovf_bytes);
uint64_t ovf_cap_elems(uint64_t ovf_bytes, bool stk16);
bool camera_inside(const zrt_camera* cam, const float root_c[3], float origin_bound);
bool lean_launch(const LaunchPlan& P, bool stats, bool cam_inside);
uint32_t reported_loop(int kmode);
LaunchPlan plan_launch(const SceneShape& s, const zrt_params* p);
int plan_pass(const zrt_params* p, uint32_t done, uint32_t n_samples, zrt_pass_plan* out);
int plan_adapt(const zrt_params* p, const zrt_adaptive* ad, std::vector<uint32_t>* levels);
int plan_variance(const zrt_params* p, uint32_t n, zrt_variance_plan* out);
int plan_denoise(const zrt_params* p, const zrt_denoise* dn, DenoiseLaunch* out);
int plan_reproject(const zrt_camera* prev, const zrt_params* p, zrt_reproject_plan* out);
int plan_temporal(const zrt_params* p, const zrt_temporal* tp, TemporalLaunch* out);

void flatten_scene(HostScene* c, const zrt_scene* s, bool use_bvh, int device, int qnodes = -1);
SceneShape shape_of(const HostScene& h);
}

#define ZRT_CATCH_HOST                                 \
  catch (const ::zrt::Error& e) {                      \
    return ::zrt::fail(e.code, e.what());              \
  }                                                    \
  catch (const std::bad_alloc&) {                      \
    return ::zrt::fail(ZRT_E_NOMEM, "OutOfMemory");    \
  }
```

zraytrace_amd/csrc/kernels.hpp:

```cpp
#pragma once
#include <hip/hip_runtime_api.h>

#include <cstddef>
#include <cstdint>

namespace zrt {
struct alignas(16) DevMaterial {
  float r, g, b, ior;
  float u_off, v_off;
  uint32_t kind, tex_kind;
  uint32_t img_w, img_h, img_off;
  uint32_t img_u8;
};

struct KArgs {
  const float4* __restrict__ nodes;
  const float4* __restrict__ prims;
  const float4* __restrict__ shade;
  const float4* __restrict__ wnodes;
  const float4* __restrict__ qleaves;
  uint32_t n_qnodes, n_qleaves;
  const DevMaterial* __restrict__ mats;
  const float* __restrict__ texels;
  const uint32_t* __restrict__ texels8;
  uint32_t* __restrict__ att;
  float4* __restrict__ partial;
  uint32_t* __restrict__ work_counter;
  uint32_t* __restrict__ unit_cost;
  const unsigned long long* __restrict__ sync_probe;
  const uint32_t* __restrict__ tile_order;
  unsigned long long* __restrict__ wave_times;
  unsigned long long* __restrict__ counters;
  unsigned long long* __restrict__ scanlines;
  uint32_t* __restrict__ error_flag;
  float org[3], llc[3], hor[3], ver[3];
  float f_width, f_height, color_scale, inv_width, inv_height;
  uint32_t width, height, xbound, spp, max_depth;
  uint32_t tiles_x, rank, world, total_work;
  uint32_t n_list, stack_depth, n_lanes;
  uint32_t chunk, n_chunks, sync;
  uint32_t n_slots;
  uint32_t wide_stride;
  uint32_t node_f4;
  uint32_t lds_rows;
  uint32_t ref_stack;
  const uint32_t* __restrict__ leaf_of_slot;
  void* stack_ovf;
  unsigned long long seed_mix;
  uint32_t n_top;
  uint32_t lds_top_off;
  uint32_t lds_att_off;
  uint32_t att_lds_rows;
  uint32_t lds_mat_off;
  uint32_t n_mats, mats_in_lds;
  uint32_t wf_thresh;
  uint32_t lds_pool_off;
  uint32_t lds_state_off;
  uint32_t n_paths;
  uint32_t tri_rcp_fast;
  float scene_extent;
  float tri_c[3], tri_h[3];
  float paxis_m;
  const uint8_t* __restrict__ ref_sph;
  float root_c[3], origin_bound;
  uint32_t check_origins;
  uint32_t layout;
  float graze_m;
  float graze_leaf;
  float guard;
  uint64_t att_cap, ovf_cap;
};

constexpr uint32_t kErrOverflow = 1u;
constexpr uint32_t kErrLayout = 2u;
constexpr uint32_t kErrBounds = 4u;

enum { kDepthHits, kReflections, kBackground, kRays, kNodes, kTriTests, kSphereTests, kShades, kTexels,
       kLeaves, kReplays, kExcessTri, kExcessSph, kExcessHits, kNumCounters };
constexpr int kWorkSlot = 14, kErrorSlot = 15, kProfSlot = 16, kScratchSlots = 48;
constexpr int kTravTrips = 21, kLoopTrips = 22, kLaneSteps = 23;
constexpr int kGlobalNodes = 24, kUniformNodes = 25, kPrimLaneTests = 26, kUniformPrims = 27;
constexpr int kAttWrites = 28, kAttReads = 29;
constexpr int kStackOvfWrites = 30;
constexpr int kProbeTrips = 31;
constexpr int kVNodeTrips = 32, kVNodeLines = 33, kSNodeTrips = 34, kRbTrips = 35, kVPrimTrips = 36,
              kVPrimLines = 37, kSPrimTrips = 38, kVShadeTrips = 39, kAttWTrips = 40, kAttRTrips = 41,
              kVNodeCost = 42, kVPrimCost = 43;

constexpr int kBlock = 256;
constexpr uint32_t kMetricShards = 64, kMetricStride = 16, kMetricWords = kMetricShards * kMetricStride;
constexpr uint32_t kTileFrozen = 0x80000000u;

struct KernelConfig {
  uint32_t waves_wide, waves_wf, waves_pool, waves_list, waves_per_simd;
  uint32_t att_rows_lock, att_rows_wf, att_rows_pool, att_rows_list;
  uint32_t stack_rows_lock, sync_samples, probe_spp;
  uint32_t oct_copies;
  uint32_t lane_words[2];
  uint32_t block_paths;
  uint32_t layout;
  float paxis_m;
  bool lds_top, lane_lds, mats_lds_only, lock_qn, profile, lean_default, grow, sphere_slots;
  bool oct_mul24;
};
const KernelConfig& kernel_config();

void* select_kernel(int kmode, uint32_t prng, bool stats, bool stk16, bool lean);
void* probe_kernel(uint32_t prng, bool stk16);
void* trace_kernel_ptr(int mode, bool stk16);
void* features_kernel_ptr(int mode, bool stk16);

hipError_t launch_finalize(hipStream_t st, const float4* partial, float* out, uint32_t n_slots, uint32_t n_chunks,
                           uint32_t world, uint32_t rank, uint32_t tiles_x, uint32_t xbound, uint32_t height,
                           float color_scale, const unsigned long long* error_flag);
hipError_t launch_accumulate(hipStream_t st, const float4* partial, float4* accum, float* out, uint32_t n_slots,
                             uint32_t pass_chunks, uint32_t world, uint32_t rank, uint32_t tiles_x, uint32_t xbound,
                             uint32_t height, float prev_scale, float new_scale, uint32_t q_chunks,
                             const unsigned long long* error_flag, unsigned long long* metrics);
hipError_t launch_resolve(hipStream_t st, const float4* partial, float4* accum, float* out, const uint32_t* active,
                          uint32_t n_active, uint32_t my_tiles, uint32_t pass_chunks, uint32_t world, uint32_t rank,
                          uint32_t tiles_x, uint32_t xbound, uint32_t height, float prev_scale, float new_scale,
                          uint32_t q_chunks, float tolerance, uint32_t decide, uint32_t level_samples,
                          uint32_t* tile_done, const unsigned long long* error_flag, unsigned long long* metrics);
hipError_t launch_compact(hipStream_t st, const uint32_t* in, uint32_t n, const uint32_t* tile_done, uint32_t* out,
                          uint32_t* count);
hipError_t launch_assemble(hipStream_t st, const float* gathered, float* frame, const uint32_t* rank_base,
                           uint32_t world, uint32_t tiles_x, uint32_t xbound, uint32_t height, uint32_t width,
                           uint32_t total, uint32_t stride_px, uint32_t n_tiles);
hipError_t launch_variance(hipStream_t st, const float4* accum, const float2* tile_plan, float* out, uint32_t n_slots,
                           uint32_t world, uint32_t rank, uint32_t tiles_x, uint32_t xbound, uint32_t height,
                           const unsigned long long* error_flag);
hipError_t launch_assemble_plane(hipStream_t st, const float* gathered, float* frame, const uint32_t* rank_base,
                                 uint32_t world, uint32_t tiles_x, uint32_t xbound, uint32_t height, uint32_t width,
                                 uint32_t total, uint32_t stride_px, uint32_t n_tiles);
hipError_t launch_features_error(hipStream_t st, float4* out, uint64_t n_f4, const unsigned long long* error_flag);
hipError_t launch_debug_math(int fn, const float* x, const float* y, float* out, uint32_t n);
hipError_t launch_debug_division(uint64_t n, unsigned long long* counts);
hipError_t launch_debug_rng(uint32_t prng, uint64_t key, unsigned long long* out, uint32_t n);
hipError_t sort_tiles(void* temp, size_t* temp_bytes, const uint32_t* cost, uint32_t* cost_sorted, const uint32_t* ids,
                      uint32_t* order, uint32_t n, hipStream_t st);
}
```

zraytrace_amd/csrc/render.hip:

```cpp
#include <hip/hip_runtime.h>
#include <hipcub/hipcub.hpp>

#include <cstdint>
#include <type_traits>

#include "accel_build.hpp"
#include "device_math.hpp"
#include "kernels.hpp"
#include "zrt.hpp"

namespace zrt {

#ifndef ZRT_DEBUG_BOUNDS
#define ZRT_DEBUG_BOUNDS 1
#endif
template <bool STATS>
__device__ __forceinline__ bool row_ok(const KArgs& a, uint64_t idx, uint64_t cap) {
  if (!STATS || !ZRT_DEBUG_BOUNDS || idx < cap) return true;
  atomicOr(a.error_flag, kErrBounds);
  return false;
}

#ifndef ZRT_RARE_ARGS
#define ZRT_RARE_ARGS 1
// ... 2841 lines not shown
    const AttRows ar{att_l, kBlock, gl, a.n_lanes};
    V3 x = mk(0.0f, 0.0f, 0.0f), loc = x, nrm = x;
    uint32_t att = 0, pend = 0;
    if (depth_left == 0) {
      ++c_depth;
      path_end = true;
    } else {
      if (STATS) ++c_rays;
      RayT r;
      r.ox = o.x; r.oy = o.y; r.oz = o.z;
      r.dx = d.x; r.dy = d.y; r.dz = d.z;
      r.rcp_det = a.tri_rcp_fast;
      r.gm = a.graze_m;
      r.gl = a.graze_leaf;
      r.gk = a.guard;
      inv_dir(d.x, d.y, d.z, r.ix, r.iy, r.iz);
      float best_t = __builtin_inff();
      int best = -1;
      for (uint32_t i = 0; i < a.n_list; ++i) {
        const uint32_t tag = __float_as_uint(cshade[i].w);
        if (tag >> 31) {
          if (STATS) ++c_tri;
          tri_test_v<false>(cprims[3 * i], cprims[3 * i + 1], cprims[3 * i + 2], (int)i, r, best_t, best);
        } else {
          if (STATS) ++c_sph;
          sphere_test<false>(cprims[3 * i], (int)i, r, best_t, best);
        }
      }
      if (ZRT_LIST_MERGE)
        shade_hit_a<STATS>(a, mats, rng, best, best_t, o, d, path_end, sky, L, c_bg, c_shade, c_tex, x, loc, nrm, att,
                           pend);
      else
        shade_step<STATS>(a, mats, ar, rng, best, best_t, o, d, depth_left, path_end, sky, L, c_bg, c_refl, c_shade,
                          c_tex, coh);
    }
    bool cam = false;
    if (path_end) {
      const V3 col = sky ? att_product<STATS>(a, mats, ar, a.max_depth - depth_left, L, coh) : L;
      acc_r += col.x;
      acc_g += col.y;
      acc_b += col.z;
      in_sample = false;
      if (++sample == s_end) {
        a.partial[slot] = make_float4(acc_r, acc_g, acc_b, 0.0f);
        has = false;
      } else if (ZRT_LIST_MERGE) {
        const uint64_t offset = (uint64_t)py * a.width + px;
        rng.init(((offset << 16) | (uint64_t)sample) + a.seed_mix);
        const float u = dev::div_known((float)px + rand_float(rng) - 0.5f, a.f_width, a.inv_width);
        const float v = dev::div_known((float)py + rand_float(rng) - 0.5f, a.f_height, a.inv_height);
        x = sub(add(add(mk(a.llc[0], a.llc[1], a.llc[2]), scale(mk(a.hor[0], a.hor[1], a.hor[2]), u)),
                    scale(mk(a.ver[0], a.ver[1], a.ver[2]), v)),
                mk(a.org[0], a.org[1], a.org[2]));
        cam = true;
        in_sample = true;
      }
    }
    if (ZRT_LIST_MERGE && (pend != 0u || cam)) {
      const V3 nd = unit(x);
      if (cam) {
        o = mk(a.org[0], a.org[1], a.org[2]);
        d = nd;
        depth_left = a.max_depth;
      } else if (pend == 1u || dot(nd, nrm) > 0.0f) {
        ++c_refl;
        if (depth_left > 1) {
          const uint32_t i = a.max_depth - depth_left;
          if (i < a.att_lds_rows) {
            ar.lds[i * ar.lds_stride] = att;
          } else {
            const uint64_t k = (uint64_t)(i - a.att_lds_rows) * ar.g_stride + ar.g_index;
            if (row_ok<STATS>(a, k, a.att_cap)) a.att[k] = att;
            if (STATS) ++coh.attw;
          }
        }
        o = loc;
        d = nd;
        --depth_left;
      } else {
        acc_r += 0.0f;
        acc_g += 0.0f;
        acc_b += 0.0f;
        in_sample = false;
        if (++sample == s_end) {
          a.partial[slot] = make_float4(acc_r, acc_g, acc_b, 0.0f);
          has = false;
        }
      }
    }
    if (a.scanlines) {
      scanline_add(a, py, 0, c_depth - dh0);
      scanline_add(a, py, 1, c_refl - rf0);
      scanline_add(a, py, 2, c_bg - bg0);
    }
  }
  if (!a.scanlines) {
    wave_add_u64(&a.counters[kDepthHits], c_depth);
    wave_add_u64(&a.counters[kReflections], c_refl);
    wave_add_u64(&a.counters[kBackground], c_bg);
  }
  if (STATS) {
    wave_add_u64(&a.counters[kRays], c_rays);
    wave_add_u64(&a.counters[kTriTests], c_tri);
    wave_add_u64(&a.counters[kSphereTests], c_sph);
    wave_add_u64(&a.counters[kShades], c_shade);
    wave_add_u64(&a.counters[kTexels], c_tex);
    wave_add_u64(&a.counters[kLoopTrips], c_loops);
    wave_add_u64(&a.counters[kLaneSteps], c_lsteps);
    coh.flush(a.counters);
  }
}

#ifndef ZRT_ATT_ROWS_LIST
#define ZRT_ATT_ROWS_LIST 24
#endif
#ifndef ZRT_ATT_ROWS_LOCK
#define ZRT_ATT_ROWS_LOCK 4
#endif
#ifndef ZRT_ATT_ROWS_WF
#define ZRT_ATT_ROWS_WF 12
#endif
#ifndef ZRT_WAVES_WF
#define ZRT_WAVES_WF 4
#endif

#ifndef ZRT_WAVES_POOL
#define ZRT_WAVES_POOL 4
#endif
#ifndef ZRT_ATT_ROWS_POOL
#define ZRT_ATT_ROWS_POOL 3
#endif

template <int MODE, int PRNG, bool STATS, class StackT, bool LEAN = false>
__global__ void __launch_bounds__(kBlock, MODE == 5 || MODE == 7 || MODE == 8 || MODE == 9 ? ZRT_WAVES_POOL
                                          : MODE == 4 ? ZRT_WAVES_WF
                                          : MODE == 3 ? ZRT_WAVES_WIDE
                                          : MODE == 0 || MODE == 6 ? ZRT_WAVES_LIST
                                                      : ZRT_WAVES_PER_SIMD)
    render_kernel(const KArgs a) {
  if constexpr (MODE == 6) render_loop_list<PRNG, STATS>(a);
  else if constexpr (MODE == 5) render_loop_pool<PRNG, STATS, StackT, false>(a);
  else if constexpr (MODE == 7) render_loop_pool<PRNG, STATS, StackT, true>(a);
  else if constexpr (MODE == 8) render_loop_pool<PRNG, STATS, StackT, false, true>(a);
  else if constexpr (MODE == 9) render_loop_pool<PRNG, STATS, StackT, true, true>(a);
  else if constexpr (MODE == 4) render_loop_wf<PRNG, STATS, StackT>(a);
  else render_loop<MODE, PRNG, STATS, StackT, false, LEAN>(a);
}

template <int PRNG, class StackT>
__global__ void __launch_bounds__(kBlock, ZRT_WAVES_WIDE) schedule_probe_kernel(const KArgs a) {
  render_loop<3, PRNG, false, StackT, true>(a);
}

template <int MODE, class StackT>
__device__ __forceinline__ void closest_hit(const KArgs& a, const V3 o, const V3 d, StackT* stk, float4* lds_top,
                                            uint32_t gl, float& best_t, int& best) {
  RayT r;
  r.ox = o.x; r.oy = o.y; r.oz = o.z;
  r.dx = d.x; r.dy = d.y; r.dz = d.z;
  r.rcp_det = a.tri_rcp_fast;
  r.gm = a.graze_m;
  r.gl = a.graze_leaf;
  r.gk = a.guard;
  inv_dir(d.x, d.y, d.z, r.ix, r.iy, r.iz);
  best_t = __builtin_inff();
  best = -1;
  uint32_t c_nodes = 0, c_leaves = 0, c_tri = 0, c_sph = 0;
  if (MODE == 0) {
    for (uint32_t i = 0; i < a.n_list; ++i) {
      if (__float_as_uint(a.shade[i].w) >> 31) tri_test<false>(a.prims, (int)i, r, best_t, best);
      else sphere_test<false>(a.prims[3 * i], (int)i, r, best_t, best);
    }
  } else if (MODE == 3) {
    uint32_t c_replays = 0;
    Coh coh;
    traverse_wide<false, StackT, true>(a, r, stk, lds_top, gl, best_t, best, c_nodes, c_leaves, c_tri, c_sph, c_replays,
                                       coh);
  } else if (MODE == 8) {
    uint32_t c_replays = 0;
    Coh coh;
    traverse_wide_q<false, StackT>(a, r, stk, lds_top, gl, best_t, best, c_nodes, c_leaves, c_tri, c_sph, c_replays,
                                   coh);
  } else {
    traverse_bvh<MODE == 1, false>(a, r, stk, best_t, best, c_nodes, c_tri, c_sph);
  }
}

template <int MODE, class StackT>
__global__ void __launch_bounds__(kBlock) trace_kernel(const KArgs a, const float* __restrict__ rays, uint32_t n,
                                                       float* __restrict__ out_t, int32_t* __restrict__ out_slot) {
  extern __shared__ __attribute__((aligned(16))) char lds_raw[];
  StackT* stk = reinterpret_cast<StackT*>(lds_raw) + threadIdx.x;
  float4* lds_top = reinterpret_cast<float4*>(lds_raw + a.lds_top_off);
  if ((MODE == 3 || MODE == 8) && !layout_ok(a)) return;
  if ((MODE == 3 || MODE == 8) && ZRT_LDS_TOP) fill_lds_top(a, lds_top);
  const uint32_t gl = blockIdx.x * kBlock + threadIdx.x;
  if (gl >= n) return;
  const float* q = rays + 6ull * gl;
  const V3 d = unit(mk(q[3], q[4], q[5]));
  float best_t;
  int best;
  closest_hit<MODE, StackT>(a, mk(q[0], q[1], q[2]), d, stk, lds_top, gl, best_t, best);
  out_t[gl] = best < 0 ? __builtin_inff() : best_t;
  out_slot[gl] = best;
}

template <int MODE, class StackT>
__global__ void __launch_bounds__(kBlock) features_kernel(const KArgs a, const uint32_t* __restrict__ slot_prim,
                                                          float4* __restrict__ out) {
  extern __shared__ __attribute__((aligned(16))) char lds_raw[];
  StackT* stk = reinterpret_cast<StackT*>(lds_raw) + threadIdx.x;
  float4* lds_top = reinterpret_cast<float4*>(lds_raw + a.lds_top_off);
  if ((MODE == 3 || MODE == 8) && !layout_ok(a)) return;
  if ((MODE == 3 || MODE == 8) && ZRT_LDS_TOP) fill_lds_top(a, lds_top);
  const uint32_t gl = blockIdx.x * kBlock + threadIdx.x;
  const uint32_t tiles_w = (a.width + 7u) / 8u;
  const uint32_t tile = gl >> 6, p = gl & 63u;
  const uint32_t px = (tile % tiles_w) * 8u + (p & 7u), py = (tile / tiles_w) * 8u + (p >> 3);
  if (px >= a.width || py >= a.height) return;
  float4* dst = out + 2ull * ((uint64_t)py * a.width + px);
  if (px >= a.xbound) {
    dst[0] = make_float4(0.0f, 0.0f, 0.0f, 0.0f);
    dst[1] = make_float4(0.0f, 0.0f, 0.0f, 0.0f);
    return;
  }
  const float u = (float)px / a.f_width;
  const float v = (float)py / a.f_height;
  const V3 llc = mk(a.llc[0], a.llc[1], a.llc[2]);
  const V3 hor = mk(a.hor[0], a.hor[1], a.hor[2]);
  const V3 ver = mk(a.ver[0], a.ver[1], a.ver[2]);
  const V3 o = mk(a.org[0], a.org[1], a.org[2]);
  const V3 d = unit(sub(add(add(llc, scale(hor, u)), scale(ver, v)), o));
  float best_t;
  int best;
  closest_hit<MODE, StackT>(a, o, d, stk, lds_top, gl, best_t, best);
  if (best < 0) {
    const V3 bg = background(d);
    dst[0] = make_float4(0.0f, 0.0f, 0.0f, 0.0f);
    dst[1] = make_float4(bg.x, bg.y, bg.z, 0.0f);
    return;
  }
  uint32_t c_shade = 0, c_tex = 0;
  Coh coh;
  HitRec h;
  hit_record<false, false>(a, a.mats, best, best_t, o, d, c_shade, c_tex, coh, h);
  const uint32_t code = h.mkind == ZRT_MAT_DIELECTRIC ? kAttOne : albedo_code<false>(h.mat, h.tag & 0x7fffffffu, h.tu, h.tv);
  const V3 alb = att_value<false>(a, a.mats, code);
  dst[0] = make_float4(h.normal.x, h.normal.y, h.normal.z, best_t);
  dst[1] = make_float4(alb.x, alb.y, alb.z, __uint_as_float(slot_prim[best] + 1u));
}

__global__ void features_error_kernel(float4* __restrict__ out, uint64_t n_f4,
                                      const unsigned long long* __restrict__ error_flag) {
  if (*error_flag == 0ull) return;
  const float q = __builtin_nanf("");
  for (uint64_t i = (uint64_t)blockIdx.x * blockDim.x + threadIdx.x; i < n_f4; i += (uint64_t)gridDim.x * blockDim.x)
    out[i] = make_float4(q, q, q, q);
}

__global__ void finalize_kernel(const float4* __restrict__ partial, float* __restrict__ out,
                                uint32_t n_slots, uint32_t n_chunks, uint32_t world, uint32_t rank,
                                uint32_t tiles_x, uint32_t xbound, uint32_t height, float color_scale,
                                const unsigned long long* __restrict__ error_flag) {
  const uint32_t i = blockIdx.x * blockDim.x + threadIdx.x;
  if (i >= n_slots) return;
  const uint32_t lt = i >> 6, p = i & 63u;
  const uint32_t t = lt * world + rank;
  const uint32_t px = (t % tiles_x) * 8u + (p & 7u);
  const uint32_t py = (t / tiles_x) * 8u + (p >> 3);
  float r = 0.0f, g = 0.0f, b = 0.0f;
  if (*error_flag != 0ull) {
    r = g = b = __builtin_nanf("");
  } else if (px < xbound && py < height) {
    for (uint32_t j = 0; j < n_chunks; ++j) {
      const float4 v = partial[(size_t)j * n_slots + i];
      r += v.x;
      g += v.y;
      b += v.z;
    }
    r *= color_scale;
    g *= color_scale;
    b *= color_scale;
  }
  out[3ull * i + 0] = r;
  out[3ull * i + 1] = g;
  out[3ull * i + 2] = b;
}

__device__ __forceinline__ uint32_t png_channel_dev(float c) {
  const float v = 255.999f * c;
  const float m = v < 255.0f ? v : 255.0f;
  return uint32_t(0.0f > m ? 0.0f : m);
}

__global__ void accumulate_kernel(const float4* __restrict__ partial, float4* __restrict__ accum,
                                  float* __restrict__ out, uint32_t n_slots, uint32_t pass_chunks, uint32_t world,
                                  uint32_t rank, uint32_t tiles_x, uint32_t xbound, uint32_t height, float prev_scale,
                                  float new_scale, uint32_t q_chunks, const unsigned long long* __restrict__ error_flag,
                                  unsigned long long* __restrict__ metrics) {
  const uint32_t i = blockIdx.x * blockDim.x + threadIdx.x;
  const bool live = i < n_slots;
  const uint32_t lt = i >> 6, p = i & 63u;
  const uint32_t t = lt * world + rank;
  const uint32_t px = (t % tiles_x) * 8u + (p & 7u);
  const uint32_t py = (t / tiles_x) * 8u + (p >> 3);
  float r = 0.0f, g = 0.0f, b = 0.0f;
// ... 214 lines not shown
  out[i] = var;
}

__global__ void debug_math_kernel(int fn, const float* __restrict__ x, const float* __restrict__ y,
                                  float* __restrict__ out, uint32_t n) {
  const uint32_t i = blockIdx.x * blockDim.x + threadIdx.x;
  if (i >= n) return;
  const float a = x[i], b = y ? y[i] : 0.0f;
  float s, c, r;
  switch (fn) {
    case 0: dev::sincos_z(a, &s, &c); r = s; break;
    case 1: dev::sincos_z(a, &s, &c); r = c; break;
    case 2: r = dev::acos_z(a); break;
    case 3: r = dev::atan_z(a); break;
    case 4: r = dev::sqrt_rn(a); break;
    case 5: r = dev::atan2_z(a, b); break;
    case 6: r = dev::pow5_z(a); break;
    case 8: r = dev::rcp_rn(a); break;
    case 9: r = dev::div_rn(a, b); break;
    default: r = a / b; break;
  }
  out[i] = r;
}

__device__ __forceinline__ uint32_t mix32(uint64_t x) {
  x ^= x >> 33;
  x *= 0xff51afd7ed558ccdull;
  x ^= x >> 33;
  x *= 0xc4ceb9fe1a85ec53ull;
  x ^= x >> 33;
  return uint32_t(x);
}
__device__ __forceinline__ bool same_f(float x, float y) {
  return __float_as_uint(x) == __float_as_uint(y) || (x != x && y != y);
}
__device__ __forceinline__ float wild_float(uint32_t h, uint32_t h2) {
  switch (h2 & 15) {
    case 0: return __uint_as_float(h & 0x807fffffu);
    case 1: return __uint_as_float((h & 0x807fffffu) | 0x7f800000u);
    case 2: return __uint_as_float((h & 0x80ffffffu) | (((h2 >> 4) & 3u) << 23) | 0x3f000000u);
    default: return __uint_as_float(h);
  }
}
__global__ void debug_division_kernel(uint64_t n, unsigned long long* __restrict__ counts) {
  const uint64_t tid = uint64_t(blockIdx.x) * blockDim.x + threadIdx.x;
  const uint64_t stride = uint64_t(gridDim.x) * blockDim.x;
  uint32_t c0 = 0, c1 = 0, c2 = 0, c3 = 0, c4 = 0;
  for (uint64_t i = tid; i < (1ull << 32); i += stride) {
    const float b = __uint_as_float(uint32_t(i));
    c0 += same_f(dev::rcp_rn(b), 1.0f / b) ? 0u : 1u;
    c0 += same_f(dev::sqrt_rn(b), __builtin_sqrtf(b)) ? 0u : 1u;
  }
  for (uint64_t i = tid; i < n; i += stride) {
    const uint32_t h0 = mix32(8 * i), h1 = mix32(8 * i + 1), h2 = mix32(8 * i + 2), h3 = mix32(8 * i + 3);
    const uint32_t h4 = mix32(8 * i + 4), h5 = mix32(8 * i + 5);
    float a = wild_float(h0, h2), b = wild_float(h1, h2 >> 8);
    if ((h3 & 3) == 0) {
      const float k = float(int(h3 >> 20) + 1) * 0.0009765625f;
      a = __uint_as_float(__float_as_uint(b * k) + int((h3 >> 2) & 7) - 3);
    }
    c1 += same_f(dev::div_rn(a, b), a / b) ? 0u : 1u;
    const int e0 = int(h4 & 255) - 128;
    V3 v;
    float* vp = &v.x;
    for (int k = 0; k < 3; ++k) {
      const uint32_t hk = mix32(8 * i + 6 + uint64_t(k) * 0x100000000ull);
      const int e = e0 + int((hk >> 24) & 31) - 16;
      const uint32_t bexp = uint32_t(e + 127 < 1 ? 0 : e + 127 > 254 ? 254 : e + 127);
      float x = __uint_as_float((hk & 0x807fffffu) | (bexp << 23));
      if (((h5 >> (4 * k)) & 15) == 0) x = (hk & 1) ? -0.0f : 0.0f;
      if (((h5 >> (4 * k)) & 15) == 1) x = __uint_as_float(hk & 0x800fffffu);
      vp[k] = x;
    }
    const float l = __builtin_sqrtf(v.x * v.x + v.y * v.y + v.z * v.z);
    const V3 u = unit(v);
    c2 += (same_f(u.x, v.x / l) && same_f(u.y, v.y / l) && same_f(u.z, v.z / l) && same_f(unit_y(v), v.y / l)) ? 0u : 1u;
    float ix, iy, iz;
    inv_dir(v.x, v.y, v.z, ix, iy, iz);
    c3 += (same_f(ix, 1.0f / v.x) && same_f(iy, 1.0f / v.y) && same_f(iz, 1.0f / v.z)) ? 0u : 1u;
    inv_dir(u.x, u.y, u.z, ix, iy, iz);
    c3 += (same_f(ix, 1.0f / u.x) && same_f(iy, 1.0f / u.y) && same_f(iz, 1.0f / u.z)) ? 0u : 1u;
    const float w = float((h0 & 0xffffu) | 1u) + float((h1 >> 16) & 0xfffeu);
    const float fw = w > 65535.0f ? 65535.0f : w;
    const float px = float(h2 & 0xffffu) * ((h3 >> 30) ? 1.0f : 0.0f);
    const float r = __uint_as_float((0x7fu << 23) | (h4 >> 9)) - 1.0f;
    const float num = px + r - 0.5f;
    c4 += same_f(dev::div_core(num, fw, 1.0f / fw), num / fw) ? 0u : 1u;
  }
  if (c0) atomicAdd(&counts[0], (unsigned long long)c0);
  if (c1) atomicAdd(&counts[1], (unsigned long long)c1);
  if (c2) atomicAdd(&counts[2], (unsigned long long)c2);
  if (c3) atomicAdd(&counts[3], (unsigned long long)c3);
  if (c4) atomicAdd(&counts[4], (unsigned long long)c4);
}

template <int PRNG>
__global__ void debug_rng_kernel(uint64_t key, unsigned long long* out, uint32_t n) {
  if (blockIdx.x != 0 || threadIdx.x != 0) return;
  Rng<PRNG> r;
  r.init(key);
  for (uint32_t i = 0; i < n; ++i) out[i] = r.next();
}

namespace {
template <int MODE, int PRNG, bool STATS, class StackT, bool LEAN = false>
void* kernel_ptr() {
  return reinterpret_cast<void*>(&render_kernel<MODE, PRNG, STATS, StackT, LEAN>);
}

template <int PRNG, bool STATS>
void* select_kernel_ps(int mode, bool stk16) {
  if (mode == 0) return kernel_ptr<0, PRNG, STATS, uint16_t>();
  if (mode == 6) return kernel_ptr<6, PRNG, STATS, uint16_t>();
  if (mode == 1) return stk16 ? kernel_ptr<1, PRNG, STATS, uint16_t>() : kernel_ptr<1, PRNG, STATS, uint32_t>();
  if (mode == 3) return stk16 ? kernel_ptr<3, PRNG, STATS, uint16_t>() : kernel_ptr<3, PRNG, STATS, uint32_t>();
  if (mode == 4) return stk16 ? kernel_ptr<4, PRNG, STATS, uint16_t>() : kernel_ptr<4, PRNG, STATS, uint32_t>();
  if (mode == 5) return stk16 ? kernel_ptr<5, PRNG, STATS, uint16_t>() : kernel_ptr<5, PRNG, STATS, uint32_t>();
  if (mode == 7) return stk16 ? kernel_ptr<7, PRNG, STATS, uint16_t>() : kernel_ptr<7, PRNG, STATS, uint32_t>();
  if (mode == 8) return stk16 ? kernel_ptr<8, PRNG, STATS, uint16_t>() : kernel_ptr<8, PRNG, STATS, uint32_t>();
  if (mode == 9) return stk16 ? kernel_ptr<9, PRNG, STATS, uint16_t>() : kernel_ptr<9, PRNG, STATS, uint32_t>();
  return stk16 ? kernel_ptr<2, PRNG, STATS, uint16_t>() : kernel_ptr<2, PRNG, STATS, uint32_t>();
}
}
#ifdef ZRT_ISA_KERNEL
void* select_kernel(int, uint32_t, bool, bool, bool) { return kernel_ptr<ZRT_ISA_KERNEL>(); }
#else
void* select_kernel(int mode, uint32_t prng, bool stats, bool stk16, bool lean) {
  if (lean) {
    if (mode != 3 || stats) throw Error(ZRT_E_UNSUPPORTED, "no lean kernel for this loop");
    if (prng == ZRT_PRNG_XOSHIRO256)
      return stk16 ? kernel_ptr<3, ZRT_PRNG_XOSHIRO256, false, uint16_t, true>()
                   : kernel_ptr<3, ZRT_PRNG_XOSHIRO256, false, uint32_t, true>();
    return stk16 ? kernel_ptr<3, ZRT_PRNG_XOROSHIRO128, false, uint16_t, true>()
                 : kernel_ptr<3, ZRT_PRNG_XOROSHIRO128, false, uint32_t, true>();
  }
  if (prng == ZRT_PRNG_XOSHIRO256)
    return stats ? select_kernel_ps<ZRT_PRNG_XOSHIRO256, true>(mode, stk16)
                 : select_kernel_ps<ZRT_PRNG_XOSHIRO256, false>(mode, stk16);
  return stats ? select_kernel_ps<ZRT_PRNG_XOROSHIRO128, true>(mode, stk16)
               : select_kernel_ps<ZRT_PRNG_XOROSHIRO128, false>(mode, stk16);
}
#endif

#ifdef ZRT_ISA_KERNEL
#define ZRT_STK(K, ...) ((void)stk16, static_cast<void*>(nullptr))
#else
#define ZRT_STK(K, ...) (stk16 ? reinterpret_cast<void*>(&K<__VA_ARGS__, uint16_t>) \
                               : reinterpret_cast<void*>(&K<__VA_ARGS__, uint32_t>))
#endif
void* probe_kernel(uint32_t prng, bool stk16) {
  return prng == ZRT_PRNG_XOSHIRO256 ? ZRT_STK(schedule_probe_kernel, ZRT_PRNG_XOSHIRO256)
                                     : ZRT_STK(schedule_probe_kernel, ZRT_PRNG_XOROSHIRO128);
}
hipError_t sort_tiles(void* temp, size_t* temp_bytes, const uint32_t* cost, uint32_t* cost_sorted, const uint32_t* ids,
                      uint32_t* order, uint32_t n, hipStream_t st) {
  return hipcub::DeviceRadixSort::SortPairsDescending(temp, *temp_bytes, cost, cost_sorted, ids, order, int(n), 0, 32, st);
}
void* features_kernel_ptr(int mode, bool stk16) {
  return mode == 0 ? ZRT_STK(features_kernel, 0) : mode == 1 ? ZRT_STK(features_kernel, 1)
       : mode == 2 ? ZRT_STK(features_kernel, 2) : mode == 8 ? ZRT_STK(features_kernel, 8) : ZRT_STK(features_kernel, 3);
}
void* trace_kernel_ptr(int mode, bool stk16) {
  return mode == 0 ? ZRT_STK(trace_kernel, 0) : mode == 1 ? ZRT_STK(trace_kernel, 1)
       : mode == 2 ? ZRT_STK(trace_kernel, 2) : mode == 8 ? ZRT_STK(trace_kernel, 8) : ZRT_STK(trace_kernel, 3);
}
#undef ZRT_STK

namespace {
template <class... P, class... A>
hipError_t launch(void (*kernel)(P...), uint32_t grid, uint32_t block, hipStream_t st, A... args) {
  hipLaunchKernelGGL(kernel, dim3(grid), dim3(block), 0, st, args...);
  return hipGetLastError();
}
}
hipError_t launch_finalize(hipStream_t st, const float4* partial, float* out, uint32_t n_slots, uint32_t n_chunks,
                           uint32_t world, uint32_t rank, uint32_t tiles_x, uint32_t xbound, uint32_t height,
                           float color_scale, const unsigned long long* error_flag) {
  return launch(finalize_kernel, (n_slots + 255) / 256, 256, st, partial, out, n_slots, n_chunks, world, rank,
                    tiles_x, xbound, height, color_scale, error_flag);
}
hipError_t launch_accumulate(hipStream_t st, const float4* partial, float4* accum, float* out, uint32_t n_slots,
                             uint32_t pass_chunks, uint32_t world, uint32_t rank, uint32_t tiles_x, uint32_t xbound,
                             uint32_t height, float prev_scale, float new_scale, uint32_t q_chunks,
                             const unsigned long long* error_flag, unsigned long long* metrics) {
  return launch(accumulate_kernel, (n_slots + 255) / 256, 256, st, partial, accum, out, n_slots, pass_chunks, world,
                    rank, tiles_x, xbound, height, prev_scale, new_scale, q_chunks, error_flag, metrics);
}
hipError_t launch_resolve(hipStream_t st, const float4* partial, float4* accum, float* out, const uint32_t* active,
                          uint32_t n_active, uint32_t my_tiles, uint32_t pass_chunks, uint32_t world, uint32_t rank,
                          uint32_t tiles_x, uint32_t xbound, uint32_t height, float prev_scale, float new_scale,
                          uint32_t q_chunks, float tolerance, uint32_t decide, uint32_t level_samples,
                          uint32_t* tile_done, const unsigned long long* error_flag, unsigned long long* metrics) {
  return launch(resolve_kernel, (n_active + 3) / 4, 256, st, partial, accum, out, active, n_active, my_tiles,
                    pass_chunks, world, rank, tiles_x, xbound, height, prev_scale, new_scale, q_chunks, tolerance,
                    decide, level_samples, tile_done, error_flag, metrics);
}
hipError_t launch_compact(hipStream_t st, const uint32_t* in, uint32_t n, const uint32_t* tile_done, uint32_t* out,
                          uint32_t* count) {
  return launch(compact_kernel, 1, kCompactBlock, st, in, n, tile_done, out, count);
}
hipError_t launch_assemble(hipStream_t st, const float* gathered, float* frame, const uint32_t* rank_base,
                           uint32_t world, uint32_t tiles_x, uint32_t xbound, uint32_t height, uint32_t width,
                           uint32_t total, uint32_t stride_px, uint32_t n_tiles) {
  return launch(assemble_kernel<3>, (total + 255) / 256, 256, st, gathered, frame, rank_base, world, tiles_x, xbound,
                    height, width, total, stride_px, n_tiles);
}
hipError_t launch_variance(hipStream_t st, const float4* accum, const float2* tile_plan, float* out, uint32_t n_slots,
                           uint32_t world, uint32_t rank, uint32_t tiles_x, uint32_t xbound, uint32_t height,
                           const unsigned long long* error_flag) {
  return launch(variance_kernel, (n_slots + 255) / 256, 256, st, accum, tile_plan, out, n_slots, world, rank, tiles_x,
                    xbound, height, error_flag);
}
hipError_t launch_assemble_plane(hipStream_t st, const float* gathered, float* frame, const uint32_t* rank_base,
                                 uint32_t world, uint32_t tiles_x, uint32_t xbound, uint32_t height, uint32_t width,
                                 uint32_t total, uint32_t stride_px, uint32_t n_tiles) {
  return launch(assemble_kernel<1>, (total + 255) / 256, 256, st, gathered, frame, rank_base, world, tiles_x, xbound,
                    height, width, total, stride_px, n_tiles);
}
hipError_t launch_features_error(hipStream_t st, float4* out, uint64_t n_f4, const unsigned long long* error_flag) {
  const uint32_t grid = uint32_t(n_f4 + 255 < 4096ull * 256 ? (n_f4 + 255) / 256 : 4096);
  return launch(features_error_kernel, grid, 256, st, out, n_f4, error_flag);
}
hipError_t launch_debug_math(int fn, const float* x, const float* y, float* out, uint32_t n) {
  return launch(debug_math_kernel, (n + 255) / 256, 256, 0, fn, x, y, out, n);
}
hipError_t launch_debug_division(uint64_t n, unsigned long long* counts) {
  return launch(debug_division_kernel, 8192, 256, 0, n, counts);
}
hipError_t launch_debug_rng(uint32_t prng, uint64_t key, unsigned long long* out, uint32_t n) {
  if (prng == ZRT_PRNG_XOSHIRO256) return launch(debug_rng_kernel<ZRT_PRNG_XOSHIRO256>, 1, 64, 0, key, out, n);
  return launch(debug_rng_kernel<ZRT_PRNG_XOROSHIRO128>, 1, 64, 0, key, out, n);
}

const KernelConfig& kernel_config() {
  static const KernelConfig k = {
      ZRT_WAVES_WIDE, ZRT_WAVES_WF, ZRT_WAVES_POOL, ZRT_WAVES_LIST, ZRT_WAVES_PER_SIMD,
      ZRT_ATT_ROWS_LOCK, ZRT_ATT_ROWS_WF, ZRT_ATT_ROWS_POOL, ZRT_ATT_ROWS_LIST,
      ZRT_STACK_ROWS_LOCK, ZRT_SYNC_SAMPLES, ZRT_PROBE_SPP,
      kOctCopies,
      {LaneState<ZRT_PRNG_XOROSHIRO128>::kWords, LaneState<ZRT_PRNG_XOSHIRO256>::kWords},
      kBlockPaths,
      kKernelLayout,
      kPaxisM,
      ZRT_LDS_TOP != 0, ZRT_LANE_LDS != 0, ZRT_MATS_LDS_ONLY != 0, ZRT_LOCK_QN != 0, ZRT_PROFILE != 0,
      ZRT_LEAN_DEFAULT != 0, ZRT_GROW != 0, ZRT_SPHERE_SLOTS != 0,
      ZRT_OCT_MUL24 != 0 && ZRT_OCT_COPIES != 0,
  };
  return k;
}
}
```

Before: 58370.

## Classify all-sky tiles on host and shade them with a lightweight sky kernel

Adds a conservative host-side classifier that walks the BVH with per-tile view cones to prove an 8x8 tile can never hit geometry. Proven sky tiles are rendered by a small kernel that only evaluates the background per sample. The main render kernel gets a compacted tile order containing only general tiles, so it no longer spends traversal work and waves on empty regions. The cost is host classification time on a cache miss, extra device lists, and a second launch, plus a dependence on the classifier's error bounds being correct.

```diff
diff --git a/include/zrt.h b/include/zrt.h
--- a/include/zrt.h
+++ b/include/zrt.h
@@ -421,6 +421,9 @@
                           uint32_t* lean);
 int zrt_debug_qnodes(const zrt_scene* scene, uint64_t* n_checked);
 int zrt_debug_octant_offsets(uint32_t stride_f4, uint32_t n_top, uint32_t node_f4);
+#define ZRT_TILE_SKY 0x80000000u
+int zrt_debug_tile_classes(const zrt_scene* scene, const zrt_camera* camera, const zrt_params* params,
+                           uint32_t* classes, uint32_t cap, uint32_t* n_tiles, uint32_t* n_sky, double* margins);
 
 #ifdef __cplusplus
 }
diff --git a/zraytrace_amd/__init__.py b/zraytrace_amd/__init__.py
--- a/zraytrace_amd/__init__.py
+++ b/zraytrace_amd/__init__.py
@@ -647,6 +647,23 @@
     return bool(out.value)
 
 
+ZRT_TILE_SKY = 0x80000000
+
+
+def debug_tile_classes(scene, camera, params):
+    view = scene.view if isinstance(scene, LoadedScene) else scene
+    p = params.abi()
+    n, n_sky = C.c_uint32(), C.c_uint32()
+    m = (C.c_double * 4)()
+    check(lib().zrt_debug_tile_classes(view, C.byref(camera), C.byref(p), None, 0, C.byref(n), C.byref(n_sky), m))
+    out = np.zeros(max(1, n.value), dtype=np.uint32)
+    check(lib().zrt_debug_tile_classes(view, C.byref(camera), C.byref(p), out.ctypes.data_as(C.POINTER(C.c_uint32)),
+                                       n.value, C.byref(n), C.byref(n_sky), m))
+    out = out[:n.value]
+    assert int((out == ZRT_TILE_SKY).sum()) == n_sky.value
+    return out, dict(sphere_reach=m[0], tri_reach=m[1], k_ao=m[2], k_c=m[3])
+
+
 def debug_qnodes(scene) -> int:
     view = scene.view if isinstance(scene, LoadedScene) else scene
     n = C.c_uint64()
diff --git a/zraytrace_amd/_ffi.py b/zraytrace_amd/_ffi.py
--- a/zraytrace_amd/_ffi.py
+++ b/zraytrace_amd/_ffi.py
@@ -299,6 +299,9 @@
     ("zrt_debug_lean_kernel", C.c_int, [C.POINTER(Scene), C.POINTER(Camera), C.POINTER(Params),
                                         C.POINTER(C.c_uint32)]),
     ("zrt_debug_qnodes", C.c_int, [C.POINTER(Scene), C.POINTER(C.c_uint64)]),
+    ("zrt_debug_tile_classes", C.c_int, [C.POINTER(Scene), C.POINTER(Camera), C.POINTER(Params),
+                                         C.POINTER(C.c_uint32), C.c_uint32, C.POINTER(C.c_uint32),
+                                         C.POINTER(C.c_uint32), C.POINTER(C.c_double)]),
     ("zrt_debug_octant_offsets", C.c_int, [C.c_uint32, C.c_uint32, C.c_uint32]),
 ]
 
diff --git a/zraytrace_amd/csrc/context.cpp b/zraytrace_amd/csrc/context.cpp
--- a/zraytrace_amd/csrc/context.cpp
+++ b/zraytrace_amd/csrc/context.cpp
@@ -216,6 +216,7 @@
   HIPCHK(sort_tiles(pr.sort_temp.p, &bytes, pr.tile_cost.p, pr.cost_sorted.p, pr.tile_ids.p, pr.tile_order.p, my_tiles,
                     st));
   a.tile_order = pr.tile_order.p;
+  ++pr.order_gen;
   return true;
 }
 
@@ -285,6 +286,7 @@
   HIPCHK(hipGetDeviceProperties(&prop, c->device));
   c->cu_count = prop.multiProcessorCount;
   upload_scene(c->scene, h);
+  build_sky_scene(&c->sky.scene, h);
   c->scratch.alloc(kScratchSlots);
   return c;
 }
@@ -339,6 +341,8 @@
   uint32_t sync = 0;
   bool order_cache = true;
   bool auto_sync = true;
+  bool sky_tiles = true;
+  bool sky_by_render = false;
   bool cap_rows = false;
   double row_cap = 1.0;
 };
@@ -351,6 +355,8 @@
   v.order_cache = !(oc && std::atoi(oc) == 0);
   const char* as = std::getenv("ZRT_AUTO_SYNC");
   v.auto_sync = !v.sync && !(as && std::atoi(as) == 0);
+  v.sky_tiles = sky_tiles_wanted();
+  if (const char* e = std::getenv("ZRT_SKY_TILES")) v.sky_by_render = std::atoi(e) == 2;
   if (const char* e = std::getenv("ZRT_DEBUG_ROW_CAP")) {
     v.cap_rows = true;
     v.row_cap = std::atof(e);
@@ -515,6 +521,61 @@
   return schedule;
 }
 
+uint32_t split_sky(zrt_ctx* c, const Frame& f, const LaunchEnv& env, KArgs& a) {
+  const zrt_params* p = f.p;
+  SkySplit& sp = c->sky;
+  if (!env.sky_tiles || f.adapt || f.my_tiles == 0 || !sp.scene.ok || !sky_split_allowed(f.plan, p, f.cam_inside))
+    return 0;
+  const OrderKey key{*f.cam, p->width, p->height, p->max_depth, p->rank, p->world_size, p->traversal,
+                     f.plan.guard_on ? 1u : 0u, f.my_tiles};
+  const bool hit = sp.valid && std::memcmp(&key, &sp.key, sizeof(key)) == 0 && (env.order_cache || !f.first);
+  if (!hit) {
+    sp.valid = false;
+    const double t0 = now_ms();
+    classify_tiles(sp.scene, f.cam, p, &sp.cls, &sp.n_sky);
+    if (env.debug)
+      std::fprintf(stderr, "zrt launch: %u of %u tiles all sky, classified in %.2f ms\n", sp.n_sky, f.my_tiles,
+                   now_ms() - t0);
+    sp.sky_host.clear();
+    sp.gen_host.clear();
+    for (uint32_t lt = 0; lt < f.my_tiles; ++lt) (sp.cls[lt] == kTileSky ? sp.sky_host : sp.gen_host).push_back(lt);
+    if (sp.n_sky) {
+      if (sp.cls_dev.n < f.my_tiles) {
+        HIPCHK(hipStreamSynchronize(f.st));
+        sp.cls_dev.alloc(f.my_tiles);
+        sp.sky_list.alloc(f.my_tiles);
+        sp.gen_list.alloc(f.my_tiles);
+        sp.gen_sorted.alloc(f.my_tiles);
+        sp.count.alloc(1);
+      }
+      const auto up = [&](DevBuf<uint32_t>& d, const std::vector<uint32_t>& h) {
+        if (!h.empty()) HIPCHK(hipMemcpyAsync(d.p, h.data(), h.size() * sizeof(uint32_t), hipMemcpyHostToDevice, f.st));
+      };
+      up(sp.cls_dev, sp.cls);
+      up(sp.sky_list, sp.sky_host);
+      up(sp.gen_list, sp.gen_host);
+      HIPCHK(hipStreamSynchronize(f.st));
+    }
+    sp.sorted_valid = false;
+    sp.key = key;
+    sp.valid = true;
+  }
+  if (sp.n_sky == 0) return 0;
+  const uint32_t n_gen = f.my_tiles - sp.n_sky;
+  if (a.tile_order) {
+    if (!sp.sorted_valid || sp.sorted_gen != c->probe.order_gen) {
+      HIPCHK(launch_compact(f.st, c->probe.tile_order.p, f.my_tiles, sp.cls_dev.p, sp.gen_sorted.p, sp.count.p));
+      sp.sorted_gen = c->probe.order_gen;
+      sp.sorted_valid = true;
+    }
+    a.tile_order = sp.gen_sorted.p;
+  } else {
+    a.tile_order = sp.gen_list.p;
+  }
+  a.total_work = uint32_t(uint64_t(n_gen) * f.pass.pass_chunks);
+  return sp.n_sky;
+}
+
 void optional_outputs(zrt_ctx* c, const Frame& f, const FrameSize& z, const LaunchEnv& env, bool schedule, KArgs& a) {
   a.sync_probe = schedule && f.plan.kmode == 3 && env.auto_sync ? c->probe.scratch.p : nullptr;
   if (f.p->flags & ZRT_FLAG_SCANLINES) {
@@ -538,13 +599,26 @@
   }
 }
 
-void enqueue(zrt_ctx* c, const Frame& f, const FrameSize& z, KArgs& a) {
+void enqueue(zrt_ctx* c, const Frame& f, const FrameSize& z, const LaunchEnv& env, KArgs& a, uint32_t n_sky) {
   const zrt_params* p = f.p;
   const Geometry& g = f.g;
   const uint32_t n_chunks = f.pass.pass_chunks, n_slots = f.my_tiles * 64u;
   unsigned long long* err = c->scratch.p + kErrorSlot;
   HIPCHK(hipEventRecord(c->ev.e0, f.st));
-  if (z.work > 0) {
+  if (n_sky > 0) {
+    KArgs sa = a;
+    sa.tile_order = c->sky.sky_list.p;
+    sa.total_work = uint32_t(uint64_t(n_sky) * n_chunks);
+    const uint32_t grid = std::max(1u, std::min(uint32_t(c->cu_count) * 8u, (sa.total_work + kBlock / 64 - 1) / (kBlock / 64)));
+    void* args[] = {&sa};
+    if (env.sky_by_render) {
+      HIPCHK(hipLaunchKernel(f.kfn, dim3(z.grid), dim3(kBlock), args, f.plan.lp.bytes, f.st));
+      HIPCHK(hipMemsetAsync(c->scratch.p + kWorkSlot, 0, sizeof(unsigned long long), f.st));
+    } else {
+      HIPCHK(hipLaunchKernel(sky_kernel_ptr(p->prng, f.diag), dim3(grid), dim3(kBlock), args, 0, f.st));
+    }
+  }
+  if (a.total_work > 0) {
     void* args[] = {&a};
     HIPCHK(hipLaunchKernel(f.kfn, dim3(z.grid), dim3(kBlock), args, f.plan.lp.bytes, f.st));
   }
@@ -579,7 +653,7 @@
                         f.st));
 }
 
-void finish(zrt_ctx* c, const Frame& f, const FrameSize& z, const KArgs& a, bool schedule) {
+void finish(zrt_ctx* c, const Frame& f, const FrameSize& z, const KArgs& a, bool schedule, uint32_t n_sky) {
   HIPCHK(hipMemcpyAsync(c->render.err.get(), c->scratch.p + kErrorSlot, sizeof(unsigned long long), hipMemcpyDeviceToHost,
                         f.st));
   HIPCHK(hipEventRecord(c->render.done, f.st));
@@ -606,6 +680,7 @@
   l.guard = a.guard;
   l.scanline_rows = (f.p->flags & ZRT_FLAG_SCANLINES) ? f.p->height : 0u;
   l.n_waves = K.profile ? z.grid * (kBlock / 64) : 0u;
+  l.sky_tiles = n_sky;
   c->last = l;
   if (f.run_pass) {
     c->run.done = f.pass.samples_after;
@@ -631,9 +706,10 @@
     if (run_pass && !f.first) rotate_events(c);
     KArgs a = fill_args(c, f, z, env);
     const bool schedule = choose_order(c, f, z, env, a);
+    const uint32_t n_sky = split_sky(c, f, env, a);
     optional_outputs(c, f, z, env, schedule, a);
-    enqueue(c, f, z, a);
-    finish(c, f, z, a, schedule);
+    enqueue(c, f, z, env, a, n_sky);
+    finish(c, f, z, a, schedule, n_sky);
     return ZRT_OK;
   }
   ZRT_CATCH_ALL
diff --git a/zraytrace_amd/csrc/context.hpp b/zraytrace_amd/csrc/context.hpp
--- a/zraytrace_amd/csrc/context.hpp
+++ b/zraytrace_amd/csrc/context.hpp
@@ -147,6 +147,19 @@
   uint32_t tile_ids_n = 0;
   OrderKey order_key{};
   bool order_valid = false;
+  uint64_t order_gen = 0;
+};
+
+struct SkySplit {
+  SkyScene scene;
+  OrderKey key{};
+  bool valid = false;
+  uint32_t n_sky = 0;
+  std::vector<uint32_t> cls, sky_host, gen_host;
+  DevBuf<uint32_t> cls_dev, sky_list, gen_list;
+  DevBuf<uint32_t> gen_sorted, count;
+  uint64_t sorted_gen = 0;
+  bool sorted_valid = false;
 };
 
 struct LastLaunch {
@@ -157,6 +170,7 @@
   float guard = 0.0f;
   uint32_t scanline_rows = 0;
   uint32_t n_waves = 0;
+  uint32_t sky_tiles = 0;
 };
 
 struct AccumRun {
@@ -227,6 +241,7 @@
   zrt::DevBuf<unsigned long long> wave_times;
   zrt::DevBuf<unsigned long long> scanlines;
   zrt::Probe probe;
+  zrt::SkySplit sky;
   zrt::EvSet ev;
   zrt::Completion render;
   zrt::LastLaunch last;
diff --git a/zraytrace_amd/csrc/debug_device.cpp b/zraytrace_amd/csrc/debug_device.cpp
--- a/zraytrace_amd/csrc/debug_device.cpp
+++ b/zraytrace_amd/csrc/debug_device.cpp
@@ -13,6 +13,7 @@
     HIPCHK(hipEventSynchronize(c->render.done));
     unsigned long long h[zrt::kScratchSlots] = {0};
     HIPCHK(hipMemcpy(h, c->scratch.p, sizeof(h), hipMemcpyDeviceToHost));
+    h[zrt::kSkyTilesSlot] = c->last.sky_tiles;
     for (uint32_t i = 0; i < n && i < uint32_t(zrt::kScratchSlots); ++i) out[i] = h[i];
     return ZRT_OK;
   }
diff --git a/zraytrace_amd/csrc/debug_plans.cpp b/zraytrace_amd/csrc/debug_plans.cpp
--- a/zraytrace_amd/csrc/debug_plans.cpp
+++ b/zraytrace_amd/csrc/debug_plans.cpp
@@ -1,4 +1,6 @@
 #include <cmath>
+#include <cstdio>
+#include <cstdlib>
 #include <cstring>
 #include <string>
 
@@ -190,6 +192,37 @@
   ZRT_CATCH_HOST
 }
 
+int zrt_debug_tile_classes(const zrt_scene* scene, const zrt_camera* camera, const zrt_params* params,
+                           uint32_t* classes, uint32_t cap, uint32_t* n_tiles, uint32_t* n_sky, double* margins) {
+  if (!camera || !n_tiles || !n_sky || (cap && !classes)) return fail(ZRT_E_INVALID, "null argument");
+  *n_tiles = *n_sky = 0;
+  int rc = zrt::validate_scene(scene);
+  if (rc) return rc;
+  rc = zrt::validate_params(params);
+  if (rc) return rc;
+  try {
+    const bool use_bvh = params->bounded_volume_hierarchy != 0 && scene->n_prims > 10;
+    zrt::HostScene h;
+    zrt::flatten_scene(&h, scene, use_bvh, -1);
+    const zrt::LaunchPlan P = zrt::plan_launch(zrt::shape_of(h), params);
+    std::vector<uint32_t> cls(zrt::rank_tiles(zrt::geometry(params), params->rank, params->world_size), zrt::kTileGeneral);
+    if (margins) margins[0] = margins[1] = margins[2] = margins[3] = 0.0;
+    if (zrt::sky_tiles_wanted() &&
+        zrt::sky_split_allowed(P, params, zrt::camera_inside(camera, h.root_c, h.origin_bound))) {
+      zrt::SkyScene sky;
+      zrt::build_sky_scene(&sky, h);
+      const double t0 = zrt::now_ms();
+      zrt::classify_tiles(sky, camera, params, &cls, n_sky, margins);
+      if (std::getenv("ZRT_DEBUG_LAUNCH"))
+        std::fprintf(stderr, "zrt tile classes: %u of %zu tiles sky in %.2f ms\n", *n_sky, cls.size(), zrt::now_ms() - t0);
+    }
+    *n_tiles = uint32_t(cls.size());
+    for (uint32_t i = 0; i < cap && i < cls.size(); ++i) classes[i] = cls[i];
+    return ZRT_OK;
+  }
+  ZRT_CATCH_HOST
+}
+
 int zrt_debug_qnodes(const zrt_scene* scene, uint64_t* n_checked) {
   if (!n_checked) return fail(ZRT_E_INVALID, "null argument");
   *n_checked = 0;
diff --git a/zraytrace_amd/csrc/host.hpp b/zraytrace_amd/csrc/host.hpp
--- a/zraytrace_amd/csrc/host.hpp
+++ b/zraytrace_amd/csrc/host.hpp
@@ -107,6 +107,30 @@
 int plan_reproject(const zrt_camera* prev, const zrt_params* p, zrt_reproject_plan* out);
 int plan_temporal(const zrt_params* p, const zrt_temporal* tp, TemporalLaunch* out);
 
+constexpr uint32_t kTileGeneral = 0u, kTileSky = kTileFrozen;
+struct SkyNode {
+  double c[3], r;
+  int32_t left, right;
+};
+struct SkyPrim {
+  double c[3], r;
+  int32_t sphere_index;
+};
+struct SkyScene {
+  bool ok = false;
+  bool has_tri = false;
+  std::vector<SkyNode> nodes;
+  std::vector<SkyPrim> prims;
+  std::vector<uint32_t> spheres;
+  double k_ao = 0, k_c = 0;
+  double tri_c[3] = {0, 0, 0}, tri_r = 0;
+};
+bool sky_tiles_wanted();
+bool sky_split_allowed(const LaunchPlan& P, const zrt_params* p, bool cam_inside);
+void build_sky_scene(SkyScene* s, const HostScene& h);
+void classify_tiles(const SkyScene& s, const zrt_camera* cam, const zrt_params* p, std::vector<uint32_t>* cls,
+                    uint32_t* n_sky, double* margins = nullptr);
+
 void flatten_scene(HostScene* c, const zrt_scene* s, bool use_bvh, int device, int qnodes = -1);
 SceneShape shape_of(const HostScene& h);
 }
diff --git a/zraytrace_amd/csrc/kernels.hpp b/zraytrace_amd/csrc/kernels.hpp
--- a/zraytrace_amd/csrc/kernels.hpp
+++ b/zraytrace_amd/csrc/kernels.hpp
@@ -87,6 +87,8 @@
               kVPrimLines = 37, kSPrimTrips = 38, kVShadeTrips = 39, kAttWTrips = 40, kAttRTrips = 41,
               kVNodeCost = 42, kVPrimCost = 43;
 
+constexpr int kSkyTilesSlot = 47;
+
 constexpr int kBlock = 256;
 constexpr uint32_t kMetricShards = 64, kMetricStride = 16, kMetricWords = kMetricShards * kMetricStride;
 constexpr uint32_t kTileFrozen = 0x80000000u;
@@ -107,6 +109,7 @@
 
 void* select_kernel(int kmode, uint32_t prng, bool stats, bool stk16, bool lean);
 void* probe_kernel(uint32_t prng, bool stk16);
+void* sky_kernel_ptr(uint32_t prng, bool stats);
 void* trace_kernel_ptr(int mode, bool stk16);
 void* features_kernel_ptr(int mode, bool stk16);
 
diff --git a/zraytrace_amd/csrc/render.hip b/zraytrace_amd/csrc/render.hip
--- a/zraytrace_amd/csrc/render.hip
+++ b/zraytrace_amd/csrc/render.hip
@@ -3017,6 +3017,43 @@
   render_loop<3, PRNG, false, StackT, true>(a);
 }
 
+template <int PRNG, bool STATS>
+__global__ void __launch_bounds__(kBlock) sky_kernel(const KArgs a) {
+  const uint32_t lane = __lane_id();
+  const uint32_t n_waves = gridDim.x * (kBlock / 64);
+  const V3 llc = mk(a.llc[0], a.llc[1], a.llc[2]);
+  const V3 hor = mk(a.hor[0], a.hor[1], a.hor[2]);
+  const V3 ver = mk(a.ver[0], a.ver[1], a.ver[2]);
+  const V3 o = mk(a.org[0], a.org[1], a.org[2]);
+  uint32_t c_bg = 0;
+  for (uint32_t u = blockIdx.x * (kBlock / 64) + (threadIdx.x >> 6); u < a.total_work; u += n_waves) {
+    const uint32_t ord = u / a.n_chunks, g = u - ord * a.n_chunks;
+    const uint32_t lt = a.tile_order[ord];
+    const uint32_t t = lt * a.world + a.rank;
+    const uint32_t px = (t % a.tiles_x) * 8u + (lane & 7u), py = (t / a.tiles_x) * 8u + (lane >> 3);
+    const uint32_t first = g * a.chunk, end = min(first + a.chunk, a.spp);
+    float acc_r = 0.0f, acc_g = 0.0f, acc_b = 0.0f;
+    if (px < a.xbound && py < a.height) {
+      const uint64_t offset = (uint64_t)py * a.width + px;
+      for (uint32_t sample = first; sample < end; ++sample) {
+        Rng<PRNG> rng;
+        rng.init(((offset << 16) | (uint64_t)sample) + a.seed_mix);
+        const float su = dev::div_known((float)px + rand_float(rng) - 0.5f, a.f_width, a.inv_width);
+        const float sv = dev::div_known((float)py + rand_float(rng) - 0.5f, a.f_height, a.inv_height);
+        const V3 d = unit(sub(add(add(llc, scale(hor, su)), scale(ver, sv)), o));
+        const V3 L = background(d);
+        acc_r += L.x;
+        acc_g += L.y;
+        acc_b += L.z;
+      }
+      c_bg += end - first;
+    }
+    a.partial[g * a.n_slots + lt * 64u + lane] = make_float4(acc_r, acc_g, acc_b, 0.0f);
+  }
+  wave_add_u64(&a.counters[kBackground], c_bg);
+  if (STATS) wave_add_u64(&a.counters[kRays], c_bg);
+}
+
 template <int MODE, class StackT>
 __device__ __forceinline__ void closest_hit(const KArgs& a, const V3 o, const V3 d, StackT* stk, float4* lds_top,
                                             uint32_t gl, float& best_t, int& best) {
@@ -3537,6 +3574,17 @@
   return prng == ZRT_PRNG_XOSHIRO256 ? ZRT_STK(schedule_probe_kernel, ZRT_PRNG_XOSHIRO256)
                                      : ZRT_STK(schedule_probe_kernel, ZRT_PRNG_XOROSHIRO128);
 }
+void* sky_kernel_ptr(uint32_t prng, bool stats) {
+#ifdef ZRT_ISA_KERNEL
+  return nullptr;
+#else
+  if (prng == ZRT_PRNG_XOSHIRO256)
+    return stats ? reinterpret_cast<void*>(&sky_kernel<ZRT_PRNG_XOSHIRO256, true>)
+                 : reinterpret_cast<void*>(&sky_kernel<ZRT_PRNG_XOSHIRO256, false>);
+  return stats ? reinterpret_cast<void*>(&sky_kernel<ZRT_PRNG_XOROSHIRO128, true>)
+               : reinterpret_cast<void*>(&sky_kernel<ZRT_PRNG_XOROSHIRO128, false>);
+#endif
+}
 hipError_t sort_tiles(void* temp, size_t* temp_bytes, const uint32_t* cost, uint32_t* cost_sorted, const uint32_t* ids,
                       uint32_t* order, uint32_t n, hipStream_t st) {
   return hipcub::DeviceRadixSort::SortPairsDescending(temp, *temp_bytes, cost, cost_sorted, ids, order, int(n), 0, 32, st);
diff --git a/zraytrace_amd/csrc/tile_class.cpp b/zraytrace_amd/csrc/tile_class.cpp
--- /dev/null
+++ b/zraytrace_amd/csrc/tile_class.cpp
@@ -0,0 +1,349 @@
+#include <algorithm>
+#include <atomic>
+#include <cmath>
+#include <cstdlib>
+#include <cstring>
+#include <thread>
+
+#include "host.hpp"
+
+namespace zrt {
+namespace {
+constexpr double kU = 0x1p-24;
+constexpr uint32_t kMaxSkyNodes = 1u << 21;
+constexpr uint32_t kTileBudget = 512;
+constexpr uint32_t kBlockBudget = 4096;
+
+struct V {
+  double x, y, z;
+};
+inline V operator-(V a, V b) { return {a.x - b.x, a.y - b.y, a.z - b.z}; }
+inline V operator+(V a, V b) { return {a.x + b.x, a.y + b.y, a.z + b.z}; }
+inline V operator*(V a, double s) { return {a.x * s, a.y * s, a.z * s}; }
+inline double dot(V a, V b) { return a.x * b.x + a.y * b.y + a.z * b.z; }
+inline V cross(V a, V b) { return {a.y * b.z - a.z * b.y, a.z * b.x - a.x * b.z, a.x * b.y - a.y * b.x}; }
+inline double len(V a) { return std::sqrt(dot(a, a)); }
+inline V vec(const zrt_vec3& v) { return {double(v.x), double(v.y), double(v.z)}; }
+inline bool finite3(V a) { return std::isfinite(a.x) && std::isfinite(a.y) && std::isfinite(a.z); }
+
+struct Cone {
+  V axis;
+  double c, s;
+  bool ok;
+};
+
+struct Classifier {
+  const SkyScene& S;
+  V o, llc, hor, ver;
+  double W, H;
+  uint32_t xbound, height, tiles_x, tiles_y, rank, world;
+  double eps;
+  double reach_tri, reach_inner;
+  std::vector<double> sphere_r;
+  std::vector<uint32_t>* cls;
+  uint32_t n_sky = 0;
+  std::vector<std::vector<int32_t>> frontier;
+  std::vector<int32_t> stack;
+
+  Cone cone_of(uint32_t tx0, uint32_t ty0, uint32_t tx1, uint32_t ty1) const {
+    const double x_lo = double(tx0 * 8u) - 0.5, x_hi = double(std::min(tx1 * 8u, xbound) - 1u) + 0.5;
+    const double y_lo = double(ty0 * 8u) - 0.5, y_hi = double(std::min(ty1 * 8u, height) - 1u) + 0.5;
+    const double us[2] = {x_lo / W, x_hi / W}, vs[2] = {y_lo / H, y_hi / H};
+    V d[4], sum{0, 0, 0};
+    for (int i = 0; i < 4; ++i) {
+      const V p = llc + hor * us[i & 1] + ver * vs[i >> 1] - o;
+      const double l = len(p);
+      if (!(l > 0.0)) return Cone{{0, 0, 1}, 0, 1, false};
+      d[i] = p * (1.0 / l);
+      sum = sum + d[i];
+    }
+    const double ls = len(sum);
+    if (!(ls > 1e-3)) return Cone{{0, 0, 1}, 0, 1, false};
+    Cone k;
+    k.axis = sum * (1.0 / ls);
+    double c = 1.0;
+    for (int i = 0; i < 4; ++i) c = std::min(c, dot(k.axis, d[i]));
+    const double s = std::sqrt(std::max(0.0, 1.0 - c * c));
+    k.c = c - eps * s - eps * eps - 1e-12;
+    k.ok = k.c > 0.1;
+    k.s = std::sqrt(std::max(0.0, 1.0 - k.c * k.c));
+    return k;
+  }
+  bool touches(const Cone& k, V c, double R) const {
+    const V w = c - o;
+    const double d2 = dot(w, w);
+    if (!(d2 > R * R)) return true;
+    const double dist = std::sqrt(d2), sa = R / dist, ca = std::sqrt(1.0 - sa * sa);
+    return !(dot(k.axis, w) / dist < k.c * ca - k.s * sa - 1e-12);
+  }
+  bool inside_a_sphere(const Cone& k) const {
+    if (S.spheres.size() > 16) return false;
+    for (const uint32_t slot : S.spheres) {
+      const SkyPrim& q = S.prims[slot];
+      const V w = V{q.c[0], q.c[1], q.c[2]} - o;
+      const double dist = len(w), r = 0.999 * q.r;
+      if (!(dist > r)) continue;
+      const double sa = r / dist, ca = std::sqrt(1.0 - sa * sa);
+      if (sa > k.s && dot(k.axis, w) / dist > ca * k.c + sa * k.s) return true;
+    }
+    return false;
+  }
+  bool prim_touches(const Cone& k, int32_t ref) const {
+    const SkyPrim& p = S.prims[uint32_t(-ref - 1) >> 1];
+    if (p.sphere_index >= 0) return touches(k, V{p.c[0], p.c[1], p.c[2]}, sphere_r[size_t(p.sphere_index)]);
+    if (p.r < 0.0) return false;
+    return touches(k, V{p.c[0], p.c[1], p.c[2]}, p.r + reach_tri);
+  }
+
+  void mark(uint32_t tx0, uint32_t ty0, uint32_t tx1, uint32_t ty1) {
+    for (uint32_t ty = ty0; ty < ty1; ++ty)
+      for (uint32_t tx = tx0; tx < tx1; ++tx) {
+        const uint32_t t = ty * tiles_x + tx;
+        if (t % world != rank) continue;
+        (*cls)[t / world] = kTileSky;
+        ++n_sky;
+      }
+  }
+  bool owns_any(uint32_t tx0, uint32_t ty0, uint32_t tx1, uint32_t ty1) const {
+    if (world == 1 || tx1 - tx0 >= world) return true;
+    for (uint32_t ty = ty0; ty < ty1; ++ty)
+      for (uint32_t tx = tx0; tx < tx1; ++tx)
+        if ((ty * tiles_x + tx) % world == rank) return true;
+    return false;
+  }
+
+  void block(uint32_t tx0, uint32_t ty0, uint32_t tx1, uint32_t ty1, size_t depth) {
+    if (!owns_any(tx0, ty0, tx1, ty1)) return;
+    const bool single = tx1 - tx0 == 1 && ty1 - ty0 == 1;
+    const Cone k = cone_of(tx0, ty0, tx1, ty1);
+    if (depth + 1 >= frontier.size()) return;
+    const std::vector<int32_t>& in = frontier[depth];
+    std::vector<int32_t>& out = frontier[depth + 1];
+    out.clear();
+    if (!k.ok) {
+      if (single) return;
+      out = in;
+    } else if (inside_a_sphere(k)) {
+      return;
+    } else {
+      uint32_t tests = 0;
+      const uint32_t budget = single ? kTileBudget : kBlockBudget;
+      stack.assign(in.rbegin(), in.rend());
+      while (!stack.empty()) {
+        if (tests >= budget) {
+          if (single) return;
+          out.insert(out.end(), stack.begin(), stack.end());
+          break;
+        }
+        const int32_t n = stack.back();
+        stack.pop_back();
+        ++tests;
+        if (n < 0) {
+          if (!prim_touches(k, n)) continue;
+          if (single) return;
+          out.push_back(n);
+          continue;
+        }
+        const SkyNode& nd = S.nodes[size_t(n)];
+        const V c{nd.c[0], nd.c[1], nd.c[2]};
+        if (!touches(k, c, nd.r + reach_inner)) continue;
+        if (!single) {
+          const V w = c - o;
+          if (nd.r + reach_inner < 0.5 * k.s * len(w)) {
+            out.push_back(n);
+            continue;
+          }
+        }
+        stack.push_back(nd.right);
+        stack.push_back(nd.left);
+      }
+    }
+    if (out.empty()) {
+      mark(tx0, ty0, tx1, ty1);
+      return;
+    }
+    if (single) return;
+    const uint32_t mx = tx1 - tx0 > 1 ? tx0 + (tx1 - tx0) / 2 : tx1, my = ty1 - ty0 > 1 ? ty0 + (ty1 - ty0) / 2 : ty1;
+    block(tx0, ty0, mx, my, depth + 1);
+    if (mx < tx1) block(mx, ty0, tx1, my, depth + 1);
+    if (my < ty1) block(tx0, my, mx, ty1, depth + 1);
+    if (mx < tx1 && my < ty1) block(mx, my, tx1, ty1, depth + 1);
+  }
+};
+}
+
+bool sky_tiles_wanted() {
+  const char* e = std::getenv("ZRT_SKY_TILES");
+  return !(e && std::atoi(e) == 0);
+}
+
+bool sky_split_allowed(const LaunchPlan& P, const zrt_params* p, bool cam_inside) {
+  return P.kmode == 3 && p->max_depth >= 1 && (p->flags & (ZRT_FLAG_SCANLINES | ZRT_FLAG_GUARD)) == 0 && cam_inside;
+}
+
+void build_sky_scene(SkyScene* s, const HostScene& h) {
+  *s = SkyScene{};
+  if (!h.use_bvh || h.n_nodes == 0 || h.n_nodes > kMaxSkyNodes) return;
+  const uint32_t n_slots = uint32_t(h.prims.size() / 3);
+  s->prims.resize(n_slots);
+  double k_ao = 0.0, k_c = 0.0;
+  V tlo{INFINITY, INFINITY, INFINITY}, thi{-INFINITY, -INFINITY, -INFINITY};
+  for (uint32_t i = 0; i < n_slots; ++i) {
+    const float4 p0 = h.prims[3 * i], p1 = h.prims[3 * i + 1], p2 = h.prims[3 * i + 2];
+    SkyPrim& q = s->prims[i];
+    uint32_t tag;
+    std::memcpy(&tag, &h.shade[i].w, 4);
+    if (!(tag >> 31)) {
+      const V c{p0.x, p0.y, p0.z};
+      const double r = std::sqrt(double(p0.w)) * (1.0 + 0x1p-22);
+      if (!finite3(c) || !std::isfinite(r)) return;
+      q.c[0] = c.x; q.c[1] = c.y; q.c[2] = c.z;
+      q.r = r;
+      q.sphere_index = int32_t(s->spheres.size());
+      s->spheres.push_back(i);
+      continue;
+    }
+    const V a{p0.x, p0.y, p0.z}, e1{p0.w, p1.x, p1.y}, e2{p1.z, p1.w, p2.x};
+    if (!finite3(a) || !finite3(e1) || !finite3(e2)) return;
+    const V b = a + e1, c = a + e2, g = (a + b + c) * (1.0 / 3.0);
+    q.c[0] = g.x; q.c[1] = g.y; q.c[2] = g.z;
+    q.r = std::max({len(a - g), len(b - g), len(c - g)}) * (1.0 + 1e-9);
+    q.sphere_index = -1;
+    const V n = cross(e1, e2);
+    const double nl = len(n);
+    if (nl * (1.0 + 1e-4) < 1e-6) {
+      q.r = -1.0;
+      continue;
+    }
+    for (const V& v : {a, b, c}) {
+      tlo = {std::min(tlo.x, v.x), std::min(tlo.y, v.y), std::min(tlo.z, v.z)};
+      thi = {std::max(thi.x, v.x), std::max(thi.y, v.y), std::max(thi.z, v.z)};
+    }
+    const double l1 = len(e1), l2 = len(e2), l3 = len(e2 - e1);
+    const double smin = std::min({nl / (l1 * l2), nl / (l1 * l3), nl / (l2 * l3)});
+    const double cmin = std::min(1e-6 / nl, 1.0);
+    k_ao = std::max(k_ao, 8.49 * kU / cmin * (2.0 + (l1 + l2) / l3) / smin);
+    k_c = std::max(k_c, (5.83 * kU * l1 * l2 / (cmin * l3) + 3.0 * kU * nl / l3) / smin);
+  }
+  if (!std::isfinite(k_ao) || !std::isfinite(k_c)) return;
+  s->k_ao = 2.0 * k_ao;
+  s->k_c = 2.0 * k_c;
+  if (tlo.x <= thi.x) {
+    const V c = (tlo + thi) * 0.5;
+    s->tri_c[0] = c.x; s->tri_c[1] = c.y; s->tri_c[2] = c.z;
+    s->tri_r = len(thi - c) * (1.0 + 1e-9);
+    s->has_tri = true;
+  }
+  s->nodes.resize(h.n_nodes);
+  for (uint32_t i = 0; i < h.n_nodes; ++i) {
+    const float4 lo = h.nodes[2 * i], hi = h.nodes[2 * i + 1];
+    const V a{lo.x, lo.y, lo.z}, b{hi.x, hi.y, hi.z};
+    if (!finite3(a) || !finite3(b)) {
+      s->nodes.clear();
+      return;
+    }
+    const V c = (a + b) * 0.5;
+    SkyNode& nd = s->nodes[i];
+    nd.c[0] = c.x; nd.c[1] = c.y; nd.c[2] = c.z;
+    nd.r = len(b - c) * (1.0 + 0x1p-20) + 0x1p-20 * (std::fabs(c.x) + std::fabs(c.y) + std::fabs(c.z));
+    std::memcpy(&nd.left, &lo.w, 4);
+    std::memcpy(&nd.right, &hi.w, 4);
+    const auto bad = [&](int32_t ref) {
+      return ref >= 0 ? uint32_t(ref) >= h.n_nodes : (uint32_t(-ref - 1) >> 1) >= n_slots;
+    };
+    if (bad(nd.left) || bad(nd.right)) {
+      s->nodes.clear();
+      return;
+    }
+  }
+  s->ok = true;
+}
+
+void classify_tiles(const SkyScene& s, const zrt_camera* cam, const zrt_params* p, std::vector<uint32_t>* cls,
+                    uint32_t* n_sky, double* m) {
+  const Geometry g = geometry(p);
+  const uint32_t mine = rank_tiles(g, p->rank, p->world_size);
+  cls->assign(mine, kTileGeneral);
+  *n_sky = 0;
+  if (m) m[0] = m[1] = m[2] = m[3] = 0.0;
+  if (!s.ok || mine == 0) return;
+  Classifier C{s};
+  C.o = vec(cam->origin);
+  C.llc = vec(cam->lower_left_corner);
+  C.hor = vec(cam->horizontal);
+  C.ver = vec(cam->vertical);
+  if (!finite3(C.o) || !finite3(C.llc) || !finite3(C.hor) || !finite3(C.ver)) return;
+  C.W = double(float(p->width));
+  C.H = double(float(p->height));
+  C.xbound = g.xbound;
+  C.height = p->height;
+  C.tiles_x = g.tiles_x;
+  C.tiles_y = g.tiles_y;
+  C.rank = p->rank;
+  C.world = p->world_size;
+  C.cls = cls;
+  const V nrm = cross(C.hor, C.ver);
+  const double nl = len(nrm);
+  if (!(nl > 0.0)) return;
+  const double h = std::fabs(dot(C.llc - C.o, nrm)) / nl;
+  const double S = len(C.llc) + len(C.hor) + len(C.ver) + len(C.o);
+  if (!(h > 0.0) || !std::isfinite(S)) return;
+  C.eps = 0x1p-20 * S / h + 0x1p-20;
+  if (!(C.eps < 1e-2)) return;
+  double reach_sph = 0.0;
+  C.sphere_r.resize(s.spheres.size());
+  for (size_t i = 0; i < s.spheres.size(); ++i) {
+    const SkyPrim& q = s.prims[s.spheres[i]];
+    const V oc = C.o - V{q.c[0], q.c[1], q.c[2]};
+    const double E = 32.0 * kU * (dot(oc, oc) + q.r * q.r);
+    C.sphere_r[i] = std::sqrt(q.r * q.r + 4.0 * E) * (1.0 + 1e-9);
+    reach_sph = std::max(reach_sph, C.sphere_r[i] - q.r);
+  }
+  C.reach_tri = 0.0;
+  if (s.has_tri) {
+    const double T = len(C.o - V{s.tri_c[0], s.tri_c[1], s.tri_c[2]}) + s.tri_r;
+    C.reach_tri = s.k_ao * T + s.k_c;
+  }
+  C.reach_inner = std::max(reach_sph, C.reach_tri);
+  if (!std::isfinite(C.reach_inner)) return;
+  if (s.has_tri && !(len(C.o - V{s.tri_c[0], s.tri_c[1], s.tri_c[2]}) > s.tri_r + C.reach_tri)) {
+    if (m) {
+      m[0] = reach_sph;
+      m[1] = C.reach_tri;
+      m[2] = s.k_ao;
+      m[3] = s.k_c;
+    }
+    return;
+  }
+  if (m) {
+    m[0] = reach_sph;
+    m[1] = C.reach_tri;
+    m[2] = s.k_ao;
+    m[3] = s.k_c;
+  }
+  C.frontier.resize(40);
+  C.frontier[0].assign(1, 0);
+  constexpr uint32_t kSquare = 32;
+  const uint32_t sq_x = (g.tiles_x + kSquare - 1) / kSquare, sq_y = (g.tiles_y + kSquare - 1) / kSquare;
+  const uint32_t n_strips = sq_x * sq_y;
+  const uint32_t n_thr = std::min({8u, std::max(1u, std::thread::hardware_concurrency()), n_strips / 4u});
+  if (n_thr <= 1) {
+    C.block(0, 0, g.tiles_x, g.tiles_y, 0);
+    *n_sky = C.n_sky;
+    return;
+  }
+  std::atomic<uint32_t> next{0}, total{0};
+  const auto work = [&]() {
+    Classifier W = C;
+    for (uint32_t i = next.fetch_add(1); i < n_strips; i = next.fetch_add(1))
+      W.block((i % sq_x) * kSquare, (i / sq_x) * kSquare, std::min(g.tiles_x, (i % sq_x + 1) * kSquare),
+              std::min(g.tiles_y, (i / sq_x + 1) * kSquare), 0);
+    total.fetch_add(W.n_sky);
+  };
+  std::vector<std::thread> pool;
+  for (uint32_t t = 1; t < n_thr; ++t) pool.emplace_back(work);
+  work();
+  for (std::thread& t : pool) t.join();
+  *n_sky = total.load();
+}
+}
```

New measurement: 64750, median of 6. +10.9%, better.
